# Zylann/godot_atmosphere_shader

Hardware: AMD Instinct MI355X
Metric: Mrays/s, direct32x8 at 1920x1080; 32 view x 8 light steps; % HBM roofline (higher is better)
Workload: dtype f32; 1 GPU; planet_atmosphere_no_clouds, 32 view x 8 light steps (direct light march); 1920x1080; demo scene, pose P_space; width=1920, height=1080, kernel=atmo_render_kernel<4, 8, 1>, gather=none (single GPU)

## Files before the change

### godot_atmosphere_shader_amd/_native.py

```python
from __future__ import annotations

import ctypes as C
import os

from .build import LIB_PATH

ATMO_OK, ATMO_E_NAME, ATMO_E_ARG, ATMO_E_STATE, ATMO_E_HIP, ATMO_E_NO_DEVICE = range(6)
VARIANT_NO_CLOUDS, VARIANT_CLOUDS, VARIANT_CLOUDS_HIGH, VARIANT_CLOUDS_HIGH_RM = range(4)
VARIANT_V1_NO_CLOUDS, VARIANT_V1_CLOUDS, VARIANT_V1_CLOUDS_HIGH = 4, 5, 6
LIGHT_LUT, LIGHT_DIRECT = 0, 1
TEX_2D_R32F, TEX_2D_R8, TEX_3D_R8, TEX_CUBE_R8 = range(4)
MEM_HOST, MEM_DEVICE = 0, 1
ABI_VERSION = 5

CORE_SYMBOLS = (
    "atmo_abi_version", "atmo_device_count", "atmo_create", "atmo_destroy", "atmo_set_param_f32", "atmo_get_param_f32",
    "atmo_set_texture", "atmo_get_texture_size", "atmo_set_sampler_lod", "atmo_bake_optical_depth",
    "atmo_generate_noise_cubemap", "atmo_read_optical_depth", "atmo_render", "atmo_render_composite", "atmo_render_tiles", "atmo_render_tiles_split", "atmo_measure_tile_costs", "atmo_set_precision",
    "atmo_set_host_double_precision", "atmo_set_target_cleared", "atmo_set_tile_feedback", "atmo_last_error_string",
)
DEBUG_SYMBOLS = (
    "atmo_set_lane_split", "atmo_debug_motion_px", "atmo_get_feedback_stats", "atmo_set_timing", "atmo_get_timing", "atmo_host_layout_cubemap", "atmo_host_layout_shape",
    "atmo_host_layout_lut", "atmo_host_cubemap_mip", "atmo_read_texture_layout", "atmo_selftest_exact_math", "atmo_debug_marched_optical_depth", "atmo_debug_log2_cr", "atmo_kernel_name", "atmo_build_id",
    "atmo_get_host_wait_stats", "atmo_get_split_stats", "atmo_debug_create_host_only", "atmo_debug_frame_constants", "atmo_debug_proxy_launch_rect",
    "atmo_debug_store_target", "atmo_debug_views_layout", "atmo_debug_views_proxy_layout", "atmo_debug_tile_order", "atmo_debug_heavy_tile_count", "atmo_debug_feedback_plan",
    "atmo_debug_decode_depth",
)
SCENE_SYMBOLS = ("atmo_render_proxy", "atmo_render_proxy_composite")
TARGET_SYMBOLS = ("atmo_target_pixel_bytes", "atmo_render_target", "atmo_render_proxy_target")
VIEWS_SYMBOLS = ("atmo_render_views",)
MAX_VIEWS = 8
VIEWS_TARGET_SYMBOLS = ("atmo_render_views_target",)
VIEWS_PROXY_SYMBOLS = ("atmo_render_views_proxy", "atmo_render_views_proxy_target")
PLANETS_SYMBOLS = ("atmo_render_planets", "atmo_plan_planets")
MAX_PLANET_DRAWS = 64
DEPTH_SYMBOLS = ("atmo_depth_texel_bytes", "atmo_render_depth_target", "atmo_render_proxy_depth_target", "atmo_render_views_depth_target",
                 "atmo_render_views_proxy_depth_target")
DEPTH_D32_SFLOAT, DEPTH_D16_UNORM, DEPTH_X8_D24_UNORM = range(3)
EXPORTED_SYMBOLS = CORE_SYMBOLS + DEBUG_SYMBOLS + SCENE_SYMBOLS + TARGET_SYMBOLS + VIEWS_SYMBOLS + VIEWS_PROXY_SYMBOLS + VIEWS_TARGET_SYMBOLS
TARGET_RGBA32F, TARGET_RGBA16F, TARGET_RGBA8_UNORM = range(3)
TARGET_RGBA8_SRGB, TARGET_BGRA8_UNORM, TARGET_BGRA8_SRGB, TARGET_A2B10G10R10_UNORM = range(16, 20)


class AtmoFrame(C.Structure):
    _fields_ = [
        ("inv_projection_matrix", C.c_float * 16),
        ("inv_view_matrix", C.c_float * 16),
        ("viewport_w", C.c_int32),
        ("viewport_h", C.c_int32),
        ("planet_center_viewspace", C.c_float * 3),
        ("sun_center_viewspace", C.c_float * 3),
        ("time", C.c_float),
        ("x0", C.c_int32),
        ("y0", C.c_int32),
        ("x1", C.c_int32),
        ("y1", C.c_int32),
    ]


class AtmoTarget(C.Structure):
    _fields_ = [
        ("pixels", C.c_void_p),
        ("format", C.c_int32),
        ("row_pitch_bytes", C.c_int32),
    ]


class AtmoView(C.Structure):
    _fields_ = [
        ("frame", AtmoFrame),
        ("depth_dev", C.c_void_p),
        ("rgba_dev", C.c_void_p),
    ]


class AtmoViewTarget(C.Structure):
    _fields_ = [
        ("frame", AtmoFrame),
        ("depth_dev", C.c_void_p),
        ("target", AtmoTarget),
    ]


class AtmoDepth(C.Structure):
    _fields_ = [
        ("texels", C.c_void_p),
        ("format", C.c_int32),
        ("row_pitch_bytes", C.c_int32),
    ]


class AtmoViewDepthTarget(C.Structure):
    _fields_ = [
        ("frame", AtmoFrame),
        ("depth", AtmoDepth),
        ("target", AtmoTarget),
    ]


class AtmoPlanetDraw(C.Structure):
    _fields_ = [
        ("ctx", C.c_void_p),
        ("frame", AtmoFrame),
        ("model_matrix", C.c_float * 16),
        ("box_size", C.c_float),
        ("depth_dev", C.c_void_p),
        ("target", AtmoTarget),
    ]


class AtmoFeedbackPlanIn(C.Structure):
    _fields_ = [
        ("fb_period", C.c_uint32), ("moving_period", C.c_uint32), ("reach_scale", C.c_float), ("instream", C.c_int32), ("axis_windows", C.c_int32),
        ("cloud_steps", C.c_int32), ("flags", C.c_int32), ("tile_h", C.c_int32), ("batch", C.c_int32), ("n", C.c_uint32), ("last_record", C.c_uint32),
        ("pending", C.c_int32), ("active", C.c_int32), ("order_born", C.c_uint32), ("order_reach_px", C.c_float), ("is_last_n", C.c_uint32),
        ("motion_px", C.c_float), ("sil_px", C.c_float * 2),
    ]


class AtmoFeedbackPlanOut(C.Structure):
    _fields_ = [
# ... 11 lines not shown
_lib = None


def load() -> C.CDLL:
    global _lib
    if _lib is not None:
        return _lib
    if not os.path.exists(LIB_PATH):
        raise RuntimeError(
            f"{LIB_PATH} is missing: the gfx950 HIP extension has not been built "
            "(python -m godot_atmosphere_shader_amd.build). There is no CPU fallback.")
    try:
        import torch
    except ImportError:
        pass
    lib = C.CDLL(LIB_PATH)
    vp, cp, ip, fp = C.c_void_p, C.c_char_p, C.c_int, C.POINTER(C.c_float)
    sig = {
        "atmo_abi_version": (ip, []),
        "atmo_device_count": (ip, []),
        "atmo_create": (ip, [ip, ip, ip, ip, ip, ip, C.POINTER(vp)]),
        "atmo_destroy": (ip, [vp]),
        "atmo_set_param_f32": (ip, [vp, cp, fp, ip]),
        "atmo_get_param_f32": (ip, [vp, cp, fp, ip]),
        "atmo_set_texture": (ip, [vp, cp, ip, ip, ip, ip, ip, vp, ip, vp]),
        "atmo_get_texture_size": (ip, [vp, cp, C.POINTER(ip), C.POINTER(ip), C.POINTER(ip), C.POINTER(ip)]),
        "atmo_set_sampler_lod": (ip, [vp, ip]),
        "atmo_read_texture_layout": (ip, [vp, cp, vp, C.c_size_t, C.POINTER(C.c_size_t), vp]),
        "atmo_host_cubemap_mip": (ip, [vp, ip, vp]),
        "atmo_generate_noise_cubemap": (ip, [vp, ip, C.c_uint32, C.c_float, ip, C.c_float, fp, ip, vp, C.POINTER(C.c_double)]),
        "atmo_bake_optical_depth": (ip, [vp, vp]),
        "atmo_read_optical_depth": (ip, [vp, vp, vp, ip, vp]),
        "atmo_render": (ip, [vp, C.POINTER(AtmoFrame), vp, vp, vp]),
        "atmo_render_composite": (ip, [vp, C.POINTER(AtmoFrame), vp, vp, vp]),
        "atmo_render_tiles": (ip, [vp, C.POINTER(AtmoFrame), vp, vp, vp, ip, vp]),
        "atmo_measure_tile_costs": (ip, [vp, C.POINTER(AtmoFrame), vp, vp, vp, vp, ip, C.POINTER(ip), C.POINTER(ip), C.POINTER(ip), C.POINTER(ip)]),
        "atmo_set_precision": (ip, [vp, ip]),
        "atmo_set_host_double_precision": (ip, [vp, ip]),
        "atmo_set_lane_split": (ip, [vp, ip]),
        "atmo_set_tile_feedback": (ip, [vp, ip]),
        "atmo_set_target_cleared": (ip, [vp, ip]),
        "atmo_debug_motion_px": (C.c_float, [C.POINTER(AtmoFrame), C.POINTER(AtmoFrame), C.c_float, ip]),
        "atmo_get_feedback_stats": (ip, [vp, C.POINTER(ip), C.POINTER(C.c_uint), C.POINTER(C.c_uint), C.POINTER(C.c_uint)]),
        "atmo_set_timing": (ip, [vp, ip]),
        "atmo_get_timing": (ip, [vp, C.POINTER(ip), C.POINTER(C.c_double)]),
        "atmo_selftest_exact_math": (ip, [vp, C.c_uint32, C.c_uint32, C.c_float, C.POINTER(C.c_uint32), C.POINTER(C.c_uint32)]),
        "atmo_debug_marched_optical_depth": (ip, [vp, ip, vp, vp, ip, vp]),
        "atmo_debug_log2_cr": (ip, [vp, ip, vp, vp]),
        "atmo_host_layout_cubemap": (ip, [vp, ip, vp]),
        "atmo_host_layout_shape": (ip, [vp, ip, vp]),
        "atmo_host_layout_lut": (ip, [vp, ip, ip, vp]),
        "atmo_kernel_name": (cp, [vp]),
        "atmo_build_id": (cp, []),
        "atmo_get_host_wait_stats": (ip, [vp, C.POINTER(C.c_uint)]),
        "atmo_get_split_stats": (ip, [vp, C.POINTER(C.c_uint), C.POINTER(C.c_uint)]),
        "atmo_render_tiles_split": (ip, [vp, C.POINTER(AtmoFrame), vp, vp, vp, ip, ip, vp]),
        "atmo_debug_create_host_only": (ip, [ip, ip, ip, ip, ip, C.POINTER(vp)]),
        "atmo_debug_frame_constants": (ip, [vp, C.POINTER(AtmoFrame), ip, C.POINTER(C.c_float), ip, C.POINTER(ip)]),
        "atmo_last_error_string": (cp, [vp]),
        "atmo_debug_proxy_launch_rect": (ip, [vp, C.POINTER(AtmoFrame), fp, C.c_float, C.POINTER(ip), C.POINTER(ip)]),
        "atmo_render_proxy": (ip, [vp, C.POINTER(AtmoFrame), fp, C.c_float, vp, vp, vp]),
        "atmo_render_proxy_composite": (ip, [vp, C.POINTER(AtmoFrame), fp, C.c_float, vp, vp, vp]),
        "atmo_target_pixel_bytes": (ip, [ip]),
        "atmo_render_target": (ip, [vp, C.POINTER(AtmoFrame), vp, C.POINTER(AtmoTarget), ip, vp]),
        "atmo_render_proxy_target": (ip, [vp, C.POINTER(AtmoFrame), fp, C.c_float, vp, C.POINTER(AtmoTarget), ip, vp]),
        "atmo_debug_store_target": (ip, [vp, ip, ip, vp, vp, C.c_size_t, vp]),
        "atmo_render_views": (ip, [vp, C.POINTER(AtmoView), ip, ip, vp]),
        "atmo_debug_views_layout": (ip, [vp, C.POINTER(AtmoView), ip, C.POINTER(ip), C.POINTER(ip)]),
        "atmo_render_views_target": (ip, [vp, C.POINTER(AtmoViewTarget), ip, ip, vp]),
        "atmo_render_views_proxy": (ip, [vp, C.POINTER(AtmoView), ip, fp, C.c_float, ip, vp]),
        "atmo_render_views_proxy_target": (ip, [vp, C.POINTER(AtmoViewTarget), ip, fp, C.c_float, ip, vp]),
        "atmo_debug_views_proxy_layout": (ip, [vp, C.POINTER(AtmoView), ip, fp, C.c_float, C.POINTER(ip), C.POINTER(ip), C.POINTER(ip)]),
        "atmo_render_planets": (ip, [C.POINTER(AtmoPlanetDraw), ip, vp]),
        "atmo_plan_planets": (ip, [C.POINTER(AtmoPlanetDraw), ip, C.POINTER(ip), C.POINTER(ip)]),
        "atmo_depth_texel_bytes": (ip, [ip]),
        "atmo_render_depth_target": (ip, [vp, C.POINTER(AtmoFrame), C.POINTER(AtmoDepth), C.POINTER(AtmoTarget), ip, vp]),
        "atmo_render_proxy_depth_target": (ip, [vp, C.POINTER(AtmoFrame), fp, C.c_float, C.POINTER(AtmoDepth), C.POINTER(AtmoTarget), ip, vp]),
        "atmo_render_views_depth_target": (ip, [vp, C.POINTER(AtmoViewDepthTarget), ip, ip, vp]),
        "atmo_render_views_proxy_depth_target": (ip, [vp, C.POINTER(AtmoViewDepthTarget), ip, fp, C.c_float, ip, vp]),
        "atmo_debug_decode_depth": (ip, [ip, vp, vp, C.c_size_t, vp]),
        "atmo_debug_tile_order": (ip, [vp, vp, ip, ip, ip, ip, vp, vp, vp, vp, C.POINTER(ip)]),
        "atmo_debug_heavy_tile_count": (ip, [vp, ip, ip, C.c_float, C.c_float, ip]),
        "atmo_debug_feedback_plan": (ip, [C.POINTER(AtmoFeedbackPlanIn), C.POINTER(AtmoFeedbackPlanOut)]),
    }
    ab_build = bool(os.environ.get("ATMO_HIP_LIB"))
    for name, (res, args) in sig.items():
        fn = getattr(lib, name, None)
        if fn is None:
            if ab_build:
                continue
            raise RuntimeError(f"libatmo_hip.so does not export {name}; rebuild it")
        fn.restype = res
        fn.argtypes = args
    have = lib.atmo_abi_version()
    if have != ABI_VERSION:
        allowed = {3, 4}
        named = os.environ.get("ATMO_HIP_LIB_ABI", "")
        if not (ab_build and named.isdigit() and int(named) == have and have in allowed):
            raise RuntimeError(f"libatmo_hip.so has ABI version {have}, this binding is written for {ABI_VERSION}; rebuild it"
                               + (f" (an older A/B library needs ATMO_HIP_LIB_ABI={have}; known-compatible: {sorted(allowed)})" if ab_build else ""))
    _lib = lib
    return lib


def check(ctx, code: int) -> None:
    if code != ATMO_OK:
        msg = load().atmo_last_error_string(ctx)
        raise AtmoError(code, msg.decode() if msg else "")
```

### godot_atmosphere_shader_amd/build.py

```python
from __future__ import annotations

import os
import shutil
import subprocess

_HERE = os.path.dirname(os.path.abspath(__file__))
CSRC = os.path.join(_HERE, "csrc")
LIB_PATH = os.environ.get("ATMO_HIP_LIB") or os.path.join(_HERE, "libatmo_hip.so")
SOURCES = ["atmo_api.hip", "atmo_kernels.hip"]
HEADERS = ["atmo_device.h", "atmo_layout.h", "atmo_feedback_plan.h", "atmo_planets_plan.h", "atmo_srgb_tables.h", os.path.join("..", "..", "include", "atmo.h"), os.path.join("..", "..", "include", "atmo_debug.h"),
           os.path.join("..", "..", "include", "atmo_scene.h"), os.path.join("..", "..", "include", "atmo_target.h"),
           os.path.join("..", "..", "include", "atmo_views.h"), os.path.join("..", "..", "include", "atmo_views_target.h"),
           os.path.join("..", "..", "include", "atmo_views_proxy.h"), os.path.join("..", "..", "include", "atmo_planets.h"),
           os.path.join("..", "..", "include", "atmo_depth.h")]

HIPCC_FLAGS = ["--offload-arch=gfx950", "-O3", "-std=c++17", "-ffp-contract=off", "-fno-slp-vectorize", "-fPIC",
               "-shared", "-Wall", "-Wno-unused-function"]


def _hipcc() -> str:
    for cand in (shutil.which("hipcc"), "/opt/rocm/bin/hipcc"):
        if cand and os.path.exists(cand):
            return cand
    raise RuntimeError("hipcc not found: the gfx950 extension cannot be built")


def needs_build() -> bool:
    if not os.path.exists(LIB_PATH):
        return True
    t = os.path.getmtime(LIB_PATH)
    deps = [os.path.join(CSRC, s) for s in SOURCES + HEADERS] + [os.path.abspath(__file__)]
    return any(os.path.getmtime(d) > t for d in deps)


def source_id() -> str:
    import hashlib

    h = hashlib.sha256()
    for name in SOURCES + HEADERS:
        with open(os.path.join(CSRC, name), "rb") as f:
            h.update(name.encode() + b"\0" + f.read())
    h.update(" ".join(HIPCC_FLAGS).encode())
    return h.hexdigest()[:16]


def build_native(force: bool = False, verbose: bool = False) -> str:
    if force or needs_build():
        cmd = [_hipcc()] + HIPCC_FLAGS + [f'-DATMO_BUILD_ID="{source_id()}"', "-o", LIB_PATH] + [os.path.join(CSRC, s) for s in SOURCES]
        if verbose:
            print(" ".join(cmd))
        subprocess.run(cmd, check=True, cwd=CSRC)
    return LIB_PATH


def build_sanitized(verbose: bool = False) -> tuple[str, str]:
    import glob

    lib = os.path.join(_HERE, "libatmo_hip_san.so")
    flags = [f for f in HIPCC_FLAGS if f != "-O3"] + ["-O1", "-g", "-fsanitize=address,undefined", "-fno-sanitize-recover=undefined",
                                                      "-fno-gpu-sanitize", "-shared-libsan"]
    cmd = [_hipcc()] + flags + ["-o", lib] + [os.path.join(CSRC, s) for s in SOURCES]
    if verbose:
        print(" ".join(cmd))
    subprocess.run(cmd, check=True, cwd=CSRC)
    rt = sorted(glob.glob("/opt/rocm/lib/llvm/lib/clang/*/lib/linux/libclang_rt.asan-x86_64.so"))
    if not rt:
        raise RuntimeError("the ASan runtime of ROCm's clang was not found")
    return lib, rt[-1]


if __name__ == "__main__":
    import sys

    if "--sanitize" in sys.argv:
        print(*build_sanitized(verbose=True))
    else:
        print(build_native(force=True, verbose=True))
```

### godot_atmosphere_shader_amd/csrc/atmo_api.hip

```cpp
#include "../../include/atmo.h"
#include "../../include/atmo_debug.h"
#include "../../include/atmo_scene.h"
#include "../../include/atmo_target.h"
#include "../../include/atmo_views.h"
#include "../../include/atmo_views_target.h"
#include "../../include/atmo_views_proxy.h"
#include "../../include/atmo_planets.h"
#include "../../include/atmo_depth.h"
#include "atmo_device.h"
#include "atmo_layout.h"
#include "atmo_feedback_plan.h"
#include "atmo_planets_plan.h"
#include "atmo_srgb_tables.h"

#include <array>
#include <cmath>
#include <cstdio>
#include <cstdlib>
#include <cstring>
#include <limits>
#include <new>
#include <string>
#include <vector>

namespace {

struct ParamDesc {
    const char *name;
    int count;
    size_t offset;
};

struct Params {
    float u_planet_radius = 1.0f;
    float u_atmosphere_height = 0.1f;
    float u_sun_position[3] = {0, 0, 0};
    float u_density = 0.2f;
    float u_scattering_strength = 20.0f;
    float u_scattering_wavelengths[3] = {700, 530, 440};
    float u_atmosphere_modulate[3] = {1, 1, 1};
    float u_atmosphere_ambient_color[3] = {0, 0, 0.002f / 12.92f};
    float u_clip_mode = 0.0f;
    float u_sphere_depth_factor = 0.0f;
    float u_cloud_density_scale = 50.0f;
    float u_cloud_bottom = 0.2f;
    float u_cloud_top = 0.5f;
    float u_cloud_blend = 0.5f;
    float u_world_to_model_matrix[16] = {1, 0, 0, 0, 0, 1, 0, 0, 0, 0, 1, 0, 0, 0, 0, 1};
    float u_cloud_shape_invert = 0.0f;
    float u_cloud_coverage_bias = 0.0f;
    float u_cloud_shape_factor = 0.8f;
    float u_cloud_shape_scale = 1.0f;
    float u_cloud_coverage_rotation[4] = {1, 0, 0, 1};
    float u_day_color0[4] = {0.21404114f, 0.60382734f, 1.0f, 1.0f};
    float u_day_color1[4] = {0.21404114f, 0.60382734f, 1.0f, 1.0f};
    float u_night_color0[4] = {0.03310477f, 0.13286832f, 0.60382734f, 1.0f};
    float u_night_color1[4] = {0.03310477f, 0.13286832f, 0.60382734f, 1.0f};
    float u_day_night_transition_scale = 2.0f;
};

#define PD(field, n) {#field, n, offsetof(Params, field)}
const ParamDesc kParams[] = {
    PD(u_planet_radius, 1), PD(u_atmosphere_height, 1), PD(u_sun_position, 3), PD(u_density, 1),
    PD(u_scattering_strength, 1), PD(u_scattering_wavelengths, 3), PD(u_atmosphere_modulate, 3),
    PD(u_atmosphere_ambient_color, 3), PD(u_clip_mode, 1), PD(u_sphere_depth_factor, 1),
    PD(u_cloud_density_scale, 1), PD(u_cloud_bottom, 1), PD(u_cloud_top, 1), PD(u_cloud_blend, 1),
    PD(u_world_to_model_matrix, 16), PD(u_cloud_shape_invert, 1), PD(u_cloud_coverage_bias, 1),
    PD(u_cloud_shape_factor, 1), PD(u_cloud_shape_scale, 1), PD(u_cloud_coverage_rotation, 4),
    PD(u_day_color0, 4), PD(u_day_color1, 4), PD(u_night_color0, 4), PD(u_night_color1, 4),
    PD(u_day_night_transition_scale, 1),
};
#undef PD

const ParamDesc *find_param(const char *name) {
    if (!name) return nullptr;
    for (const ParamDesc &d : kParams)
        if (std::strcmp(d.name, name) == 0) return &d;
    return nullptr;
}

struct DeviceBuffer {
    void *ptr = nullptr;
    size_t bytes = 0;
};

constexpr int F4_MAX_CUBE_N = 1024, F4_MAX_SHAPE_N = 64;

thread_local std::string g_create_error = "";

}

// ... 1 lines not shown
    int device = 0;
    int variant = 0;
    int flags = 0;
    int view_steps = 8, cloud_steps = 0, light_steps = 0;
    Params p;
    DeviceBuffer lut, blue, shape, cube;
    DeviceBuffer cube_f4, shape_f4;
    int f4_max_shape_n = F4_MAX_SHAPE_N;
    DeviceBuffer lut4;
    int lut_w = 0, lut_h = 0, shape_n = 0, cube_n = 0;
    int cube_levels = 0;
    DeviceBuffer cube_level_off;
    uint32_t cube_level_off_host[16] = {0};
    int sampler_lod = -1;
    DeviceBuffer staging;
    hipStream_t staging_stream = nullptr;
    bool staging_used = false;
    hipEvent_t tex_event = nullptr;
    hipStream_t tex_stream = nullptr;
    bool tex_pending = false;
    unsigned tex_version = 0;
    hipStream_t tex_waited_stream = nullptr;
    unsigned tex_waited_version = 0;
    int host_double_precision = 0;
    int target_cleared = 0;
    int lane_split = 0;
    int last_split = 1;
    int last_flags = -1;
    int tile_feedback = -1;
    struct FeedbackState {
        bool used = false;
        int tiles_x = 0, tiles_y = 0, split = 0;
        hipStream_t draw_stream = nullptr;
        DeviceBuffer cost, order[2];
        DeviceBuffer dil[2];
        AtmoFrame prev_frame;
        bool have_prev = false;
        float motion_px = 0.0f;
        float sil_px[2] = {0.0f, 0.0f};
        float order_reach_px[2] = {0.0f, 0.0f};
        unsigned order_born[2] = {0, 0};
        DeviceBuffer is_order, is_scratch;
        unsigned is_last_n = ~0u;
        DeviceBuffer order2[2], is_order2;
        uint32_t *class_totals = nullptr;
        unsigned n = 0;
        unsigned last_record = 0;
        int active = -1;
        int write = 0;
        bool pending = false;
        bool drop_pending = false;
        hipEvent_t ev_draw = nullptr, ev_order[2] = {nullptr, nullptr};
        unsigned long long last_use = 0;
        bool dirty = false;
    };
    struct GeoCache {
        float key[26] = {0};
        int rows = -1;
        uint16_t prefix[atmo::GEO_MAX_ROWS + 1];
        uint8_t first[atmo::GEO_MAX_ROWS];
        uint16_t hint[2][atmo::GEO_MAX_HINTS + 2];
    } geo;
    int geo_order = 1;
    unsigned geo_draws = 0;
    static constexpr int FB_SLOTS = 4;
    FeedbackState fb[FB_SLOTS];
    unsigned long long fb_clock = 0;
    int fb_budget = 8;
    unsigned fb_ordered_draws = 0, fb_recycled = 0, fb_sorts = 0;
    hipStream_t fb_stream = nullptr;
    hipStream_t split_stream = nullptr;
    int heavy_split = 1;
    float heavy_split_trigger = 2.0f;
    float heavy_split_trigger_moving = 2.0f;
    float heavy_split_ratio = 0.3f;
    unsigned split_draws = 0, split_tiles_last = 0;
    DeviceBuffer fb_scratch;
    unsigned fb_period = 8;
    int env_feedback = -1, env_split = 0;
    float env_reach_scale = 1.0f;
    unsigned moving_period = 2;
    int f4_footprints = 3;
    int env_lod0_cert = 1;
    int instream = 1;
    int fb_axis_windows = 1;
    uint32_t *measure_cost = nullptr;
    struct DrawStream { hipStream_t stream = nullptr; hipEvent_t last_draw = nullptr; bool recorded = false; unsigned long long last_use = 0; };
    unsigned long long draw_stream_clock = 0;
    std::vector<DrawStream> draw_streams;
    bool draw_streams_many = false;
    int draw_events = 1;
    hipEvent_t xs_event[8] = {nullptr};
    unsigned xs_next = 0;
    unsigned device_syncs = 0;
    DeviceBuffer measure_buf;
    struct TileListBuf { hipStream_t stream = nullptr; DeviceBuffer buf; bool used = false; unsigned long long last_use = 0; } tile_lists[4];
    unsigned long long tile_list_clock = 0;
#ifdef ATMO_WAVE_TRACE
    DeviceBuffer wave_trace;
    size_t wave_trace_waves = 0;
#endif
    static constexpr int VIEWS_RING = 16;
    struct ViewsSlot {
        atmo::RenderConsts *host = nullptr;
        atmo::RenderConsts *dev = nullptr;
        hipEvent_t done = nullptr;
        bool in_flight = false;
    } views_ring[VIEWS_RING];
    atmo::RenderConsts *views_host = nullptr;
    DeviceBuffer views_dev;
    unsigned views_next = 0;
    unsigned views_ring_waits = 0;
    FeedbackState views_fb;
    struct ViewsFeedbackKey {
        int flags = -1, n = 0, grid[8][2] = {{0}};
        AtmoFrame prev[8];
        float motion_px[8] = {0};
    } views_key;
    int timing = 0;
    int launch_counter = 0;
    int timed_launches = 0;
    double timed_ms = 0.0;
    std::vector<std::pair<hipEvent_t, hipEvent_t>> pending;
    std::string err;
};

namespace {

int fail(AtmoContext *ctx, int code, const std::string &msg) {
    if (ctx) ctx->err = msg; else g_create_error = msg;
    return code;
}

int hip_fail(AtmoContext *ctx, hipError_t e, const char *what) {
    return fail(ctx, ATMO_E_HIP, std::string(what) + ": " + hipGetErrorString(e));
}

#define HIP_TRY(ctx, call)                                   \
    do {                                                     \
        hipError_t e_ = (call);                              \
        if (e_ != hipSuccess) return hip_fail(ctx, e_, #call); \
    } while (0)

#define ATMO_TRY(call) do { const int rc_ = (call); if (rc_ != ATMO_OK) return rc_; } while (0)

int dev_alloc(AtmoContext *ctx, DeviceBuffer &b, size_t bytes) {
    if (b.ptr && b.bytes == bytes) return ATMO_OK;
    if (b.ptr) { (void)hipFree(b.ptr); b.ptr = nullptr; b.bytes = 0; }
    if (bytes == 0) return ATMO_OK;
    HIP_TRY(ctx, hipMalloc(&b.ptr, bytes));
    b.bytes = bytes;
    return ATMO_OK;
}

void dev_free(DeviceBuffer &b) {
    if (b.ptr) (void)hipFree(b.ptr);
    b.ptr = nullptr;
    b.bytes = 0;
}

void build_cube_footprints(const uint8_t *faces, int n, std::vector<uint32_t> &out) {
    const int fs = n + 1;
    out.assign((size_t)6 * fs * fs, 0u);
    for (int f = 0; f < 6; ++f)
        for (int j = 0; j < fs; ++j)
            for (int i = 0; i < fs; ++i) out[((size_t)f * fs + j) * fs + i] = atmo::cube_footprint_word(faces, n, f, i, j);
}

void build_shape_footprints(const uint8_t *t, int n, std::vector<uint32_t> &out) {
    out.assign((size_t)n * n * n, 0u);
    for (int k = 0; k < n; ++k)
        for (int j = 0; j < n; ++j)
            for (int i = 0; i < n; ++i) out[((size_t)k * n + j) * n + i] = atmo::shape_footprint_word(t, n, i, j, k);
}

void build_lut_apron(const float *lut, int w, int h, std::vector<float> &out) {
    const int st = w + 2;
    out.assign((size_t)st * (h + 2), 0.0f);
    for (int j = 0; j < h + 2; ++j)
        for (int i = 0; i < st; ++i) out[(size_t)j * st + i] = atmo::lut_apron_value(lut, w, h, i, j);
}

inline float pow2f(float x) { return x * x; }
inline float pow4f(float x) { return x * x * x * x; }
inline float mixf(float a, float b, float t) { return a * (1.0f - t) + b * t; }
inline float clampf(float x, float lo, float hi) { return std::fmin(std::fmax(x, lo), hi); }
inline float smoothstepf(float e0, float e1, float x) {
    float t = clampf((x - e0) / (e1 - e0), 0.0f, 1.0f);
    return t * t * (3.0f - 2.0f * t);
}

void fill_consts(const AtmoContext *ctx, const AtmoFrame *f, const float *depth, float *rgba, atmo::RenderConsts &rc) {
    const Params &p = ctx->p;
    std::memset(&rc, 0, sizeof(rc));
    std::memcpy(rc.inv_p, f->inv_projection_matrix, sizeof(rc.inv_p));
    std::memcpy(rc.inv_v, f->inv_view_matrix, sizeof(rc.inv_v));
    const float *V = f->inv_view_matrix;
    for (int r = 0; r < 3; ++r) rc.cam_pos_world[r] = V[0 + r] * 0.0f + V[4 + r] * 0.0f + V[8 + r] * 0.0f + V[12 + r] * 1.0f;
    rc.vw = (float)f->viewport_w;
    rc.vh = (float)f->viewport_h;
    rc.rcp_vw = 1.0f / rc.vw;
    rc.rcp_vh = 1.0f / rc.vh;
    rc.w = f->viewport_w; rc.h = f->viewport_h;
    rc.x0 = f->x0; rc.y0 = f->y0; rc.x1 = f->x1; rc.y1 = f->y1;
    for (int i = 0; i < 3; ++i) rc.center[i] = f->planet_center_viewspace[i];
    {
        float d[3];
        for (int i = 0; i < 3; ++i) d[i] = f->sun_center_viewspace[i] - f->planet_center_viewspace[i];
        float inv = 1.0f / std::sqrt(d[0] * d[0] + d[1] * d[1] + d[2] * d[2]);
        for (int i = 0; i < 3; ++i) rc.sun_dir[i] = d[i] * inv;
    }
    rc.planet_radius = p.u_planet_radius;
    rc.atmosphere_height = p.u_atmosphere_height;
    rc.atmosphere_radius = p.u_planet_radius + p.u_atmosphere_height;
    rc.density = p.u_density;
    rc.sphere_depth_factor = p.u_sphere_depth_factor;
    for (int i = 0; i < 3; ++i) {
        rc.coeff[i] = pow4f(400.0f / p.u_scattering_wavelengths[i]) * p.u_scattering_strength;
        rc.ambient[i] = p.u_atmosphere_ambient_color[i];
        rc.modulate[i] = p.u_atmosphere_modulate[i];
    }
    rc.view_steps = ctx->view_steps;
    rc.light_steps = ctx->light_steps;
    for (int i = 0; i < 3; ++i) {
        rc.day0[i] = p.u_day_color0[i]; rc.day1[i] = p.u_day_color1[i];
        rc.night0[i] = p.u_night_color0[i]; rc.night1[i] = p.u_night_color1[i];
    }
    rc.day_night_transition_scale = p.u_day_night_transition_scale;

    rc.clouds_bottom = p.u_planet_radius + p.u_cloud_bottom * p.u_atmosphere_height;
    rc.clouds_top = p.u_planet_radius + p.u_cloud_top * p.u_atmosphere_height;
    rc.cloud_thickness = rc.clouds_top - rc.clouds_bottom;
    rc.inv_cloud_thickness = 1.0f / rc.cloud_thickness;
    {
        const double lo = (double)rc.clouds_bottom * (double)rc.clouds_bottom * (1.0 - 2e-6);
        const double hi = (double)rc.clouds_top * (double)rc.clouds_top * (1.0 + 2e-6);
        rc.layer_r2_lo = (float)lo;
        rc.layer_r2_hi = (float)hi;
        if (!(rc.clouds_bottom > 0.0f)) rc.layer_r2_lo = 0.0f;
        if (!(rc.cloud_thickness > 0.0f) || !(rc.clouds_top > 0.0f) || !std::isfinite(rc.layer_r2_hi)) { rc.layer_r2_lo = 0.0f; rc.layer_r2_hi = INFINITY; }
    }
    rc.cloud_density_scale = p.u_cloud_density_scale;
    rc.cloud_blend = p.u_cloud_blend;
    rc.coverage_bias = p.u_cloud_coverage_bias;
    rc.shape_factor = p.u_cloud_shape_factor;
    rc.shape_scale = p.u_cloud_shape_scale;
    rc.shape_invert = (p.u_cloud_shape_invert == 1.0f) ? 1 : 0;
    {
        const float f = p.u_cloud_shape_factor;
        const float t_hi = 1.0f + 9.5367431640625e-07f;
        float a = 0.5f * (1.0f - f) + 0.0f * f, b = 0.5f * (1.0f - f) + t_hi * f;
        if (rc.shape_invert) { a = 1.0f - a; b = 1.0f - b; }
        rc.shape_lo01 = std::fmin(a, b) - 0.1f;
        rc.shape_hi01 = std::fmax(a, b) - 0.1f;
    }
    std::memcpy(rc.cov_rot, p.u_cloud_coverage_rotation, sizeof(rc.cov_rot));
    const float *A = p.u_world_to_model_matrix;
    for (int col = 0; col < 4; ++col)
        for (int row = 0; row < 4; ++row)
            rc.view_to_model[col * 4 + row] = A[0 * 4 + row] * V[col * 4 + 0] + A[1 * 4 + row] * V[col * 4 + 1] +
                                              A[2 * 4 + row] * V[col * 4 + 2] + A[3 * 4 + row] * V[col * 4 + 3];
    const float *M = rc.view_to_model;
    for (int r = 0; r < 3; ++r) {
        rc.origin_model[r] = M[0 + r] * 0.0f + M[4 + r] * 0.0f + M[8 + r] * 0.0f + M[12 + r] * 1.0f;
        rc.sun_dir_model[r] = M[0 + r] * rc.sun_dir[0] + M[4 + r] * rc.sun_dir[1] + M[8 + r] * rc.sun_dir[2] + M[12 + r] * 0.0f;
    }
    {
        const float ground = p.u_planet_radius, top = rc.clouds_top, bottom = rc.clouds_bottom;
        const float space = 0.5f * std::sqrt(1.0f - pow2f(ground / top)) * bottom;
        const float groundd = 3.0f * space;
        const float len = std::sqrt(rc.origin_model[0] * rc.origin_model[0] + rc.origin_model[1] * rc.origin_model[1] +
                                    rc.origin_model[2] * rc.origin_model[2]);
        rc.max_d = mixf(groundd, space, smoothstepf(bottom, top * 1.05f, len));
    }
    rc.cloud_steps = ctx->cloud_steps;
    rc.inv_cloud_steps = ctx->cloud_steps > 0 ? 1.0f / (float)ctx->cloud_steps : 0.0f;
    {
        const float reach = (rc.clouds_top - rc.clouds_bottom) * 0.15f;
        const float inv_steps = 1.0f / 6.0f;
        float step_len = reach * inv_steps;
        for (int i = 0; i < 6; ++i) {
            rc.rm_offset[i] = (float)i * step_len;
            rc.rm_weight[i] = step_len * p.u_cloud_density_scale;
            for (int c = 0; c < 3; ++c) rc.rm_tap[i][c] = rc.rm_offset[i] * rc.sun_dir_model[c];
            step_len *= 1.2f;
        }
    }
    rc.lut = (const float *)ctx->lut.ptr; rc.lut_w = ctx->lut_w; rc.lut_h = ctx->lut_h;
    rc.lut4 = (const float *)ctx->lut4.ptr;
    rc.blue = (const uint8_t *)ctx->blue.ptr;
    rc.shape = (const uint32_t *)ctx->shape.ptr; rc.shape_n = ctx->shape_n;
    rc.shape_log2n = -1;
    for (int b = 0; b < 10; ++b) if (ctx->shape_n == (1 << b)) rc.shape_log2n = b;
    rc.cube = (const uint32_t *)ctx->cube.ptr; rc.cube_n = ctx->cube_n;
    rc.cube_levels = ctx->cube_levels;
    rc.cube_level_off = (const uint32_t *)ctx->cube_level_off.ptr;
    rc.cube_bytes = (uint32_t)ctx->cube.bytes;
    rc.cube_f4 = (ctx->f4_footprints & 1) ? (const float *)ctx->cube_f4.ptr : nullptr;
    rc.shape_f4 = (ctx->f4_footprints & 2) ? (const float *)ctx->shape_f4.ptr : nullptr;
    rc.cube_lod_fast = (ctx->cube_n >= 1 && ctx->cube_n <= 1024 && (ctx->cube_n & (ctx->cube_n - 1)) == 0) ? 1 : 0;
    {
        rc.lod0_inv_c = std::numeric_limits<float>::infinity();
        rc.lod0_last = (float)(rc.cloud_steps - 1);
        rc.lod0_drift = (float)((rc.cloud_steps + 1) * 2.07e-7);
        const double n = (double)ctx->cube_n;
        const double a = rc.cov_rot[0], b = rc.cov_rot[2], c = rc.cov_rot[1], d = rc.cov_rot[3];
        const double fro = a * a + b * b + c * c + d * d, det = a * d - b * c;
        const double disc = fro * fro - 4.0 * det * det;
        const double sigma = std::sqrt(0.5 * (fro + std::sqrt(disc > 0.0 ? disc : 0.0))) * (1.0 + 1e-6);
        const double sigma_min = sigma > 0.0 ? std::fabs(det) / sigma : 0.0;
        const double sigma_eff = sigma > 1.0 ? sigma : 1.0;
        if (rc.cube_lod_fast && ctx->cube_n >= 4 && sigma <= 2.0 && sigma_min >= 0.5) {
            rc.lod0_inv_c = (float)(1.0 / (0.97 * 4.0 * (1.0 - 2.0 / n) * (1.0 - 2.0 / n) / (n * n * sigma_eff * sigma_eff)));
        }
        if (ctx->env_lod0_cert == 0) rc.lod0_inv_c = std::numeric_limits<float>::infinity();
    }
    {
        const float *Pm = f->inv_projection_matrix;
        const double cc = (double)rc.center[0] * rc.center[0] + (double)rc.center[1] * rc.center[1] + (double)rc.center[2] * rc.center[2];
        const double k = cc - (double)rc.atmosphere_radius * rc.atmosphere_radius;
        const bool depth_free = Pm[8] == 0.0f && Pm[9] == 0.0f && Pm[10] == 0.0f;
        rc.miss_k = (depth_free && k > 0.01 * cc && std::isfinite(k)) ? (float)(k * (1.0 - 1e-3) * (1.0 - 1e-3)) : 0.0f;
    }
    rc.depth = depth;
    rc.out = (float4 *)rgba;
    rc.out_pitch = f->x1 - f->x0;
    rc.out_x0 = f->x0;
    rc.out_y0 = f->y0;
    rc.composite = 0;
    rc.store_discards = ctx->target_cleared ? 0 : 1;
    rc.gx0 = f->x0;
    rc.gy0 = f->y0;
}

int resolve_sampler_lod(const AtmoContext *ctx, const char **why_not) {
    if (why_not) *why_not = nullptr;
    if (ctx->sampler_lod == 0 || !(ctx->flags & atmo::KF_CLOUDS) || !ctx->cube.ptr || ctx->cube_levels <= 1) return 0;
    if (!(ctx->flags & atmo::KF_PRECISE)) {
        if (why_not) *why_not = "atmo_render: the implicit cubemap LOD (atmo_set_sampler_lod 1) needs the precise cloud mode (atmo_set_precision 1)";
        return 0;
    }
    return 1;
}

int heavy_tile_count(const uint32_t *totals, int n_tiles, float ratio, float trigger, int resident_waves) {
    double life[atmo::TILE_ORDER_CLASSES], sum = 0.0;
    long long counted = 0;
    for (int k = 0; k < atmo::TILE_ORDER_CLASSES; ++k) {
        constexpr int P = atmo::TILE_ORDER_PER_OCTAVE;
        const int q = atmo::TILE_ORDER_CLASSES - 1 - k + 8 * P;
        life[k] = P == 2 ? std::ldexp(1.0, q >> 1) * ((q & 1) ? 1.5 : 1.0) * 1.2
                         : std::ldexp(1.0, q / P) * (1.0 + ((q % P) + 0.5) / P);
        if (k == atmo::TILE_ORDER_CLASSES - 1) life[k] = 0.0;
        sum += life[k] * (double)totals[k];
        counted += totals[k];
    }
    if (counted != n_tiles || sum <= 0.0) return 0;
    const double draw = sum * 2.0 / (double)resident_waves;
    int first = 0;
    while (first < atmo::TILE_ORDER_CLASSES - 1 && totals[first] == 0) ++first;
    if (!(life[first] > trigger * draw)) return 0;
    int heavy = 0;
    for (int k = 0; k < atmo::TILE_ORDER_CLASSES && life[k] > ratio * draw; ++k) heavy += (int)totals[k];
    return heavy > n_tiles / 3 ? n_tiles / 3 : heavy;
}

int choose_split(const AtmoContext *ctx, const AtmoFrame *f) {
    (void)f;
    if (ctx->flags & atmo::KF_ATMO_REF) return 1;
    if (ctx->env_split) return ctx->env_split;
    return ctx->lane_split == 2 ? 2 : 1;
}

void launch_shape(const AtmoContext *ctx, const AtmoFrame *frame, int *flags_out, int *split_out, bool *lod_out) {
    int flags = ctx->flags, split = choose_split(ctx, frame);
    if (ctx->view_steps > 32 && !(flags & (atmo::KF_LITE | atmo::KF_ATMO_REF))) {
        flags |= atmo::KF_VIEW_POS;
        split = 1;
    }
    const bool lod = resolve_sampler_lod(ctx, nullptr) != 0;
    if (lod) {
        flags |= atmo::KF_CUBE_LOD;
        if ((flags & ~atmo::KF_CLOUD_LIGHT_RM) != (atmo::KF_CUBE_LOD | atmo::KF_PRECISE | atmo::KF_CLOUDS)) split = 1;
    }
    *flags_out = flags;
    *split_out = split;
    if (lod_out) *lod_out = lod;
}

int check_frame(AtmoContext *ctx, const std::string &who, const AtmoFrame *frame, bool *empty) {
    if (!frame) return fail(ctx, ATMO_E_ARG, who + ": null frame");
    if (frame->viewport_w < 1 || frame->viewport_h < 1 || frame->viewport_w > 65536 || frame->viewport_h > 65536)
        return fail(ctx, ATMO_E_ARG, who + ": bad viewport size");
    if (frame->x0 < 0 || frame->y0 < 0 || frame->x1 > frame->viewport_w || frame->y1 > frame->viewport_h ||
        frame->x0 > frame->x1 || frame->y0 > frame->y1)
        return fail(ctx, ATMO_E_ARG, who + ": rect outside the viewport");
    *empty = frame->x0 == frame->x1 || frame->y0 == frame->y1;
    return ATMO_OK;
}
int check_draw_pointers(AtmoContext *ctx, const std::string &who, const float *depth_dev, const float *rgba_dev, bool float4_target) {
    if (!depth_dev || !rgba_dev) return fail(ctx, ATMO_E_ARG, who + ": null device pointer");
    if (float4_target && (reinterpret_cast<uintptr_t>(rgba_dev) & 15u) != 0) return fail(ctx, ATMO_E_ARG, who + ": rgba_dev must be 16-byte aligned");
    return ATMO_OK;
}
static_assert((int)ATMO_DEPTH_D32_SFLOAT == (int)atmo::DF_D32_SFLOAT && (int)ATMO_DEPTH_D16_UNORM == (int)atmo::DF_D16_UNORM &&
                  (int)ATMO_DEPTH_X8_D24_UNORM == (int)atmo::DF_X8_D24_UNORM,
              "DepthFormat == AtmoDepthFormat");
int depth_check(AtmoContext *ctx, const std::string &who, const AtmoDepth *depth, int w, int h, atmo::DepthConsts *out) {
    (void)h;
    if (!depth) return fail(ctx, ATMO_E_ARG, who + ": null depth");
    const int tb = atmo::depth_texel_bytes(depth->format);
    if (tb == 0) return fail(ctx, ATMO_E_ARG, who + ": unknown depth format " + std::to_string(depth->format));
    if (!depth->texels) return fail(ctx, ATMO_E_ARG, who + ": null depth texels");
    if ((reinterpret_cast<uintptr_t>(depth->texels) & (uintptr_t)(tb - 1)) != 0)
        return fail(ctx, ATMO_E_ARG, who + ": depth texels must be aligned to the texel size (" + std::to_string(tb) + " bytes)");
// ... 352 lines not shown
bool two_lane_form(const AtmoContext *ctx, int flags) {
    const int lod_cloud = atmo::KF_CUBE_LOD | atmo::KF_PRECISE | atmo::KF_CLOUDS;
    return ctx->heavy_split == 2 ? (flags & ~atmo::KF_CLOUD_LIGHT_RM) == lod_cloud : flags == (lod_cloud | atmo::KF_CLOUD_LIGHT_RM);
}

}

extern "C" {

int atmo_abi_version(void) { return ATMO_ABI_VERSION; }
#ifndef ATMO_BUILD_ID
#define ATMO_BUILD_ID "unstamped"
#endif
const char *atmo_build_id(void) { return ATMO_BUILD_ID; }

int atmo_device_count(void) {
    int n = 0;
    hipError_t e = hipGetDeviceCount(&n);
    if (e != hipSuccess) return -ATMO_E_NO_DEVICE;
    return n;
}

static int check_create_args(int variant, int view_steps, int cloud_steps, int light_mode, int light_steps, AtmoContext **out) {
    if (!out) return fail(nullptr, ATMO_E_ARG, "atmo_create: out is null");
    *out = nullptr;
    if (variant < ATMO_VARIANT_NO_CLOUDS || variant > ATMO_VARIANT_V1_CLOUDS_HIGH)
        return fail(nullptr, ATMO_E_ARG, "atmo_create: unknown variant");
    if (light_mode != ATMO_LIGHT_LUT && light_mode != ATMO_LIGHT_DIRECT)
        return fail(nullptr, ATMO_E_ARG, "atmo_create: unknown light mode");
    if (view_steps < 0 || view_steps > 4096 || cloud_steps < 0 || cloud_steps > 4096 || light_steps < 0 || light_steps > 4096)
        return fail(nullptr, ATMO_E_ARG, "atmo_create: step count out of range");
    if (light_mode == ATMO_LIGHT_DIRECT && light_steps < 1)
        return fail(nullptr, ATMO_E_ARG, "atmo_create: direct light mode needs light_steps >= 1");
    return ATMO_OK;
}
static void init_variant(AtmoContext *ctx, int device, int variant, int view_steps, int cloud_steps, int light_mode, int light_steps) {
    ctx->device = device;
    ctx->variant = variant;
    const bool lite = variant >= ATMO_VARIANT_V1_NO_CLOUDS;
    static const int shipped_cloud_steps[7] = {0, 32, 64, 64, 0, 32, 64};
    ctx->view_steps = view_steps > 0 ? view_steps : (lite ? 16 : 8);
    ctx->cloud_steps = shipped_cloud_steps[variant] == 0 ? 0 : (cloud_steps > 0 ? cloud_steps : shipped_cloud_steps[variant]);
    ctx->light_steps = (light_mode == ATMO_LIGHT_DIRECT && !lite) ? light_steps : 0;
    ctx->flags = 0;
    if (ctx->cloud_steps > 0) ctx->flags |= atmo::KF_CLOUDS | atmo::KF_PRECISE;
    if (lite) ctx->flags |= atmo::KF_PRECISE;
    if (variant == ATMO_VARIANT_CLOUDS_HIGH_RM) ctx->flags |= atmo::KF_CLOUD_LIGHT_RM;
    if (light_mode == ATMO_LIGHT_DIRECT && !lite) ctx->flags |= atmo::KF_LIGHT_DIRECT;
    if (lite) ctx->flags |= atmo::KF_LITE;
}

int atmo_create(int device, int variant, int view_steps, int cloud_steps, int light_mode, int light_steps,
                AtmoContext **out) {
    ATMO_TRY(check_create_args(variant, view_steps, cloud_steps, light_mode, light_steps, out));
    int n = 0;
    hipError_t e = hipGetDeviceCount(&n);
    if (e != hipSuccess || n <= 0)
        return fail(nullptr, ATMO_E_NO_DEVICE, std::string("atmo_create: no HIP device (") + hipGetErrorString(e) + ")");
    if (device < 0 || device >= n) return fail(nullptr, ATMO_E_NO_DEVICE, "atmo_create: device index out of range");
    hipDeviceProp_t prop;
    e = hipGetDeviceProperties(&prop, device);
    if (e != hipSuccess) return hip_fail(nullptr, e, "hipGetDeviceProperties");
    if (std::strncmp(prop.gcnArchName, "gfx950", 6) != 0)
        return fail(nullptr, ATMO_E_NO_DEVICE, std::string("atmo_create: device is ") + prop.gcnArchName + ", this library is built for gfx950 only");
    e = hipSetDevice(device);
    if (e != hipSuccess) return hip_fail(nullptr, e, "hipSetDevice");

    AtmoContext *ctx = new (std::nothrow) AtmoContext();
    if (!ctx) return fail(nullptr, ATMO_E_ARG, "atmo_create: out of host memory");
    init_variant(ctx, device, variant, view_steps, cloud_steps, light_mode, light_steps);

    if (const char *ev = std::getenv("ATMO_LANE_SPLIT")) ctx->env_split = ev[0] == '1' ? 1 : (ev[0] == '2' ? 2 : 0);
    if (const char *ev = std::getenv("ATMO_TILE_FEEDBACK")) ctx->env_feedback = ev[0] == '1' ? 1 : 0;
    if (const char *ev = std::getenv("ATMO_F4")) ctx->f4_footprints = std::atoi(ev) & 3;
    if (const char *ev = std::getenv("ATMO_F4_SHAPE_MAX")) ctx->f4_max_shape_n = std::atoi(ev);
    if (const char *ev = std::getenv("ATMO_LOD0_CERT")) ctx->env_lod0_cert = ev[0] == '0' ? 0 : 1;
    if (const char *ev = std::getenv("ATMO_HEAVY_SPLIT")) ctx->heavy_split = ev[0] == '0' ? 0 : (ev[0] == '2' ? 2 : 1);
    if (const char *ev = std::getenv("ATMO_HEAVY_SPLIT_RATIO")) ctx->heavy_split_ratio = (float)std::atof(ev);
    if (const char *ev = std::getenv("ATMO_HEAVY_SPLIT_TRIGGER")) ctx->heavy_split_trigger = (float)std::atof(ev);
    if (const char *ev = std::getenv("ATMO_HEAVY_SPLIT_TRIGGER_MOVING")) ctx->heavy_split_trigger_moving = (float)std::atof(ev);
    if (const char *ev = std::getenv("ATMO_DRAW_EVENTS")) ctx->draw_events = ev[0] == '0' ? 0 : (ev[0] == '2' ? 2 : 1);
    if (const char *ev = std::getenv("ATMO_TARGET_CLEARED")) ctx->target_cleared = ev[0] == '1' ? 1 : 0;
    if (const char *ev = std::getenv("ATMO_GEO_ORDER")) ctx->geo_order = ev[0] == '0' ? 0 : 1;
    if (const char *ev = std::getenv("ATMO_FB_INSTREAM")) ctx->instream = ev[0] >= '1' && ev[0] <= '2' ? ev[0] - '0' : 0;
    if (const char *ev = std::getenv("ATMO_FB_AXIS_WINDOWS")) ctx->fb_axis_windows = ev[0] == '1' ? 1 : 0;
    if (const char *ev = std::getenv("ATMO_FB_REACH_SCALE")) ctx->env_reach_scale = (float)std::atof(ev);
    if (const char *ev = std::getenv("ATMO_FB_MOVING_PERIOD")) { const int v = std::atoi(ev); ctx->moving_period = (unsigned)(v < 1 ? 1 : v); }
    if (const char *ev = std::getenv("ATMO_TILE_FEEDBACK_PERIOD")) { const int v = std::atoi(ev); ctx->fb_period = (unsigned)(v < 1 ? 1 : v); }

    int rc = dev_alloc(ctx, ctx->blue, 256 * 256);
    if (rc == ATMO_OK) {
        e = hipMemset(ctx->blue.ptr, 0, 256 * 256);
        if (e != hipSuccess) rc = hip_fail(ctx, e, "hipMemset");
    }
    if (rc != ATMO_OK) {
        g_create_error = ctx->err;
        dev_free(ctx->blue);
        delete ctx;
        return rc;
    }
    *out = ctx;
    return ATMO_OK;
}

int atmo_destroy(AtmoContext *ctx) {
    if (!ctx) return ATMO_OK;
    if (ctx->device < 0) { delete ctx; return ATMO_OK; }
    (void)hipSetDevice(ctx->device);
    drain_timing(ctx);
    dev_free(ctx->lut);
    dev_free(ctx->lut4);
    dev_free(ctx->blue);
    dev_free(ctx->shape);
    dev_free(ctx->cube);
    dev_free(ctx->cube_level_off);
    dev_free(ctx->cube_f4);
    dev_free(ctx->shape_f4);
    dev_free(ctx->staging);
    dev_free(ctx->measure_buf);
    for (AtmoContext::TileListBuf &t : ctx->tile_lists) dev_free(t.buf);
    if (ctx->tex_event) (void)hipEventDestroy(ctx->tex_event);
    for (hipEvent_t &ev : ctx->xs_event) if (ev) (void)hipEventDestroy(ev);
    for (AtmoContext::DrawStream &d : ctx->draw_streams) if (d.last_draw) (void)hipEventDestroy(d.last_draw);

    if (ctx->fb_stream) {
        (void)hipStreamSynchronize(ctx->fb_stream);
        (void)hipStreamDestroy(ctx->fb_stream);
    }
    if (ctx->split_stream) {
        (void)hipStreamSynchronize(ctx->split_stream);
        (void)hipStreamDestroy(ctx->split_stream);
    }
    for (int i = 0; i <= AtmoContext::FB_SLOTS; ++i) {
        AtmoContext::FeedbackState &f = i < AtmoContext::FB_SLOTS ? ctx->fb[i] : ctx->views_fb;
        if (f.ev_draw) (void)hipEventDestroy(f.ev_draw);
        for (int k = 0; k < 2; ++k) {
            if (f.ev_order[k]) (void)hipEventDestroy(f.ev_order[k]);
            dev_free(f.order[k]);
            dev_free(f.dil[k]);
        }
        dev_free(f.is_order);
        dev_free(f.is_scratch);
        dev_free(f.is_order2);
        for (int k = 0; k < 2; ++k) dev_free(f.order2[k]);
        if (f.class_totals) (void)hipHostFree(f.class_totals);
        dev_free(f.cost);
    }
    for (AtmoContext::ViewsSlot &v : ctx->views_ring) {
        if (v.done) { (void)hipEventSynchronize(v.done); (void)hipEventDestroy(v.done); }
    }
    if (ctx->views_host) (void)hipHostFree(ctx->views_host);
    dev_free(ctx->views_dev);
    dev_free(ctx->fb_scratch);
    delete ctx;
    return ATMO_OK;
}

int atmo_set_param_f32(AtmoContext *ctx, const char *name, const float *v, int n) {
    if (!ctx) return ATMO_E_ARG;
    if (!v) return fail(ctx, ATMO_E_ARG, "atmo_set_param_f32: value is null");
    const ParamDesc *d = find_param(name);
    if (!d) return fail(ctx, ATMO_E_NAME, std::string("atmo_set_param_f32: unknown uniform '") + (name ? name : "(null)") + "'");
    if (n != d->count)
        return fail(ctx, ATMO_E_ARG, std::string("atmo_set_param_f32: '") + name + "' takes " + std::to_string(d->count) + " floats");
    std::memcpy(reinterpret_cast<char *>(&ctx->p) + d->offset, v, sizeof(float) * n);
    return ATMO_OK;
// ... 824 lines not shown
    if (e != hipSuccess) return hip_fail(ctx, e, "atmo_debug_marched_optical_depth");
    return ATMO_OK;
}

int atmo_debug_log2_cr(AtmoContext *ctx, int n, const float *x, float *out) {
    if (!ctx) return ATMO_E_ARG;
    if (n < 1 || !x || !out) return fail(ctx, ATMO_E_ARG, "atmo_debug_log2_cr: bad argument");
    HIP_TRY(ctx, hipSetDevice(ctx->device));
    float *d = nullptr;
    HIP_TRY(ctx, hipMalloc(&d, 2 * (size_t)n * sizeof(float)));
    hipError_t e = hipMemcpy(d, x, (size_t)n * sizeof(float), hipMemcpyHostToDevice);
    if (e == hipSuccess) e = atmo::launch_log2_cr(d, d + n, n, nullptr);
    if (e == hipSuccess) e = hipMemcpy(out, d + n, (size_t)n * sizeof(float), hipMemcpyDeviceToHost);
    (void)hipFree(d);
    if (e != hipSuccess) return hip_fail(ctx, e, "atmo_debug_log2_cr");
    return ATMO_OK;
}

int atmo_debug_tile_order(AtmoContext *ctx, const uint32_t *cost, int tiles_x, int tiles_y, int rx, int ry, uint32_t *order_out, uint32_t *order2_out,
                          uint32_t *class_totals_out, uint32_t *cost_after_out, int *n_classes_out) {
    if (!ctx) return ATMO_E_ARG;
    if (!cost || !order_out) return fail(ctx, ATMO_E_ARG, "atmo_debug_tile_order: cost and order_out must not be NULL");
    if (tiles_x < 1 || tiles_y < 1 || (long long)tiles_x * tiles_y > (1ll << 22))
        return fail(ctx, ATMO_E_ARG, "atmo_debug_tile_order: the grid must be at least 1 x 1 and hold at most 2^22 tiles");
    if (rx < 0 || ry < 0 || rx > 64 || ry > 64) return fail(ctx, ATMO_E_ARG, "atmo_debug_tile_order: dilation radii are 0 .. 64 tiles");
    HIP_TRY(ctx, hipSetDevice(ctx->device));
    constexpr size_t NC = atmo::TILE_ORDER_CLASSES;
    const size_t n = (size_t)tiles_x * (size_t)tiles_y, scratch_words = atmo::tile_order_scratch_bytes() / sizeof(uint32_t);
    const size_t words = 6 * n + NC + scratch_words;
    uint32_t *d = nullptr;
    HIP_TRY(ctx, hipMalloc(&d, words * sizeof(uint32_t)));
    uint32_t *d_cost = d, *d_order = d + n, *d_order2 = d + 2 * n, *d_tmp1 = d + 4 * n, *d_tmp2 = d + 5 * n, *d_totals = d + 6 * n, *d_scratch = d_totals + NC;
    hipError_t e = hipMemset(d, 0xFF, words * sizeof(uint32_t));
    if (e == hipSuccess) e = hipMemcpy(d_cost, cost, n * sizeof(uint32_t), hipMemcpyHostToDevice);
    if (e == hipSuccess) e = atmo::launch_tile_order(d_cost, d_order, tiles_x, tiles_y, rx, ry, d_tmp1, d_tmp2, d_scratch, nullptr,
                                                     order2_out ? d_order2 : nullptr, class_totals_out ? d_totals : nullptr);
    if (e == hipSuccess) e = hipMemcpy(order_out, d_order, n * sizeof(uint32_t), hipMemcpyDeviceToHost);
    if (e == hipSuccess && order2_out) e = hipMemcpy(order2_out, d_order2, 2 * n * sizeof(uint32_t), hipMemcpyDeviceToHost);
    if (e == hipSuccess && class_totals_out) e = hipMemcpy(class_totals_out, d_totals, NC * sizeof(uint32_t), hipMemcpyDeviceToHost);
    if (e == hipSuccess && cost_after_out) e = hipMemcpy(cost_after_out, d_cost, n * sizeof(uint32_t), hipMemcpyDeviceToHost);
    (void)hipFree(d);
    if (e != hipSuccess) return hip_fail(ctx, e, "atmo_debug_tile_order");
    if (n_classes_out) *n_classes_out = (int)NC;
    return ATMO_OK;
}

int atmo_debug_heavy_tile_count(const uint32_t *class_totals, int n_classes, int n_tiles, float ratio, float trigger, int resident_waves) {
    if (!class_totals || n_classes != atmo::TILE_ORDER_CLASSES || n_tiles < 0 || resident_waves < 1)
        return -fail(nullptr, ATMO_E_ARG, "atmo_debug_heavy_tile_count: bad argument (NULL totals, a class count other than the build's, n_tiles < 0 or resident_waves < 1)");
    return heavy_tile_count(class_totals, n_tiles, ratio, trigger, resident_waves);
}

const char *atmo_kernel_name(AtmoContext *ctx) {
    if (!ctx) return "";
    if (ctx->last_flags >= 0) return atmo::render_kernel_name(ctx->last_flags, ctx->light_steps, ctx->last_split);
    int flags = 0, split = 1;
    launch_shape(ctx, nullptr, &flags, &split, nullptr);
    return atmo::render_kernel_name(flags, ctx->light_steps, split);
}

const char *atmo_last_error_string(AtmoContext *ctx) {
    if (!ctx) return g_create_error.c_str();
    return ctx->err.c_str();
}

int atmo_get_split_stats(AtmoContext *ctx, unsigned *split_draws, unsigned *heavy_tiles_last) {
    if (!ctx) return ATMO_E_ARG;
    if (split_draws) *split_draws = ctx->split_draws;
    if (heavy_tiles_last) *heavy_tiles_last = ctx->split_tiles_last;
    return ATMO_OK;
}

int atmo_get_host_wait_stats(AtmoContext *ctx, unsigned *device_syncs) {
    if (!ctx) return ATMO_E_ARG;
    if (device_syncs) *device_syncs = ctx->device_syncs;
    return ATMO_OK;
}

int atmo_debug_create_host_only(int variant, int view_steps, int cloud_steps, int light_mode, int light_steps, AtmoContext **out) {
    ATMO_TRY(check_create_args(variant, view_steps, cloud_steps, light_mode, light_steps, out));
    AtmoContext *ctx = new (std::nothrow) AtmoContext();
    if (!ctx) return fail(nullptr, ATMO_E_ARG, "atmo_debug_create_host_only: out of host memory");
    init_variant(ctx,  -1, variant, view_steps, cloud_steps, light_mode, light_steps);
    *out = ctx;
    return ATMO_OK;
}

int atmo_debug_frame_constants(AtmoContext *ctx, const AtmoFrame *frame, int cube_n, float *out, int capacity, int *count) {
    if (!ctx) return ATMO_E_ARG;
    if (!frame) return fail(ctx, ATMO_E_ARG, "atmo_debug_frame_constants: null frame");
    if (cube_n < 0 || cube_n > 4096) return fail(ctx, ATMO_E_ARG, "atmo_debug_frame_constants: bad cubemap size");
    const int saved_n = ctx->cube_n;
    ctx->cube_n = cube_n;
    AtmoFrame fixed;
    atmo::RenderConsts rc;
    fill_consts(ctx, draw_frame(ctx, frame, fixed), nullptr, nullptr, rc);
    ctx->cube_n = saved_n;
    std::vector<float> v;
    auto put = [&](const float *p, int n) { v.insert(v.end(), p, p + n); };
    auto put1 = [&](float x) { v.push_back(x); };
    put(rc.cam_pos_world, 3); put(rc.sun_dir, 3); put1(rc.atmosphere_radius); put(rc.coeff, 3);
    put1(rc.clouds_bottom); put1(rc.clouds_top); put1(rc.cloud_thickness); put1(rc.inv_cloud_thickness);
    put1(rc.layer_r2_lo); put1(rc.layer_r2_hi); put1(rc.shape_lo01); put1(rc.shape_hi01);
    put(rc.view_to_model, 16); put(rc.origin_model, 3); put(rc.sun_dir_model, 3);
    put1(rc.max_d); put1(rc.inv_cloud_steps); put(rc.rm_offset, 6); put(rc.rm_weight, 6); put(&rc.rm_tap[0][0], 18);
    put1(rc.lod0_inv_c); put1(rc.lod0_last); put1(rc.lod0_drift); put1(rc.miss_k); put1(rc.rcp_vw); put1(rc.rcp_vh);
    put1((float)rc.shape_invert); put1((float)rc.cube_lod_fast); put1((float)rc.store_discards);
    if (count) *count = (int)v.size();
    if (!out) return ATMO_OK;
    if (capacity < (int)v.size()) return fail(ctx, ATMO_E_ARG, "atmo_debug_frame_constants: buffer too small");
    std::memcpy(out, v.data(), v.size() * sizeof(float));
    return ATMO_OK;
}


static void mat4_mul_d(const double *a, const double *b, double *c) {
    for (int col = 0; col < 4; ++col)
        for (int row = 0; row < 4; ++row) {
            double acc = 0.0;
            for (int k = 0; k < 4; ++k) acc += a[k * 4 + row] * b[col * 4 + k];
            c[col * 4 + row] = acc;
        }
}
static bool mat4_inverse_d(const double *m, double *inv) {
    double a[4][8];
    for (int r = 0; r < 4; ++r)
        for (int c = 0; c < 4; ++c) { a[r][c] = m[c * 4 + r]; a[r][c + 4] = r == c ? 1.0 : 0.0; }
    for (int c = 0; c < 4; ++c) {
        int piv = c;
        for (int r = c + 1; r < 4; ++r) if (std::fabs(a[r][c]) > std::fabs(a[piv][c])) piv = r;
        if (!(std::fabs(a[piv][c]) > 0.0) || !std::isfinite(a[piv][c])) return false;
        for (int k = 0; k < 8; ++k) std::swap(a[c][k], a[piv][k]);
        const double d = a[c][c];
        for (int k = 0; k < 8; ++k) a[c][k] /= d;
        for (int r = 0; r < 4; ++r)
            if (r != c && a[r][c] != 0.0) {
                const double f = a[r][c];
                for (int k = 0; k < 8; ++k) a[r][k] -= f * a[c][k];
            }
    }
    for (int r = 0; r < 4; ++r)
        for (int c = 0; c < 4; ++c) inv[c * 4 + r] = a[r][c + 4];
    return true;
}

static int proxy_setup(AtmoContext *ctx, const char *who, const AtmoFrame *f, const float *model_matrix, float box_size, bool lod,
                       atmo::ProxyConsts &pc, int rect[4], int *tiles_x, int *tiles_y) {
    double ip[16], iv[16], m[16], mi[16], v[16], p[16], t[16], k[16], pv[16];
    for (int i = 0; i < 16; ++i) { ip[i] = f->inv_projection_matrix[i]; iv[i] = f->inv_view_matrix[i]; m[i] = model_matrix[i]; }
    if (!mat4_inverse_d(m, mi)) return fail(ctx, ATMO_E_ARG, std::string(who) + ": model_matrix is singular");
    if (!mat4_inverse_d(iv, v)) return fail(ctx, ATMO_E_ARG, std::string(who) + ": inv_view_matrix is singular");
    if (!mat4_inverse_d(ip, p)) return fail(ctx, ATMO_E_ARG, std::string(who) + ": inv_projection_matrix is singular");
    mat4_mul_d(mi, iv, t);
    mat4_mul_d(t, ip, k);
    for (int r = 0; r < 4; ++r)
        for (int c = 0; c < 4; ++c) pc.k[r][c] = (float)k[c * 4 + r];
    const double h = 0.5 * (double)box_size;
    pc.half = (float)h;
    mat4_mul_d(v, m, t);
    mat4_mul_d(p, t, pv);
    double eye[4] = {k[8], k[9], k[10], k[11]};
    bool eye_point = std::fabs(eye[3]) > 1e-12 * (std::fabs(eye[0]) + std::fabs(eye[1]) + std::fabs(eye[2]));
    if (eye_point) {
        for (int r = 0; r < 3; ++r) eye[r] /= eye[3];
    } else {
        double dn[3], df[3];
        for (int r = 0; r < 3; ++r) { dn[r] = (k[8 + r] + k[12 + r]) / (k[11] + k[15]); df[r] = k[12 + r] / k[15]; }
        if (eye[0] * (df[0] - dn[0]) + eye[1] * (df[1] - dn[1]) + eye[2] * (df[2] - dn[2]) > 0.0)
            for (int r = 0; r < 3; ++r) eye[r] = -eye[r];
    }
    const double W = f->viewport_w, H = f->viewport_h;
    double xmin = INFINITY, xmax = -INFINITY, ymin = INFINITY, ymax = -INFINITY;
    bool unbounded = false;
    for (int face = 0; face < 6; ++face) {
        const int ax = face >> 1;
        const double sg = (face & 1) ? -1.0 : 1.0;
        if (!(sg * eye[ax] > (eye_point ? h : 0.0))) continue;
        const int u = (ax + 1) % 3, w3 = (ax + 2) % 3;
        std::vector<std::array<double, 4>> poly, next;
        for (int c = 0; c < 4; ++c) {
            double mp[3];
            mp[ax] = sg * h;
            mp[u] = (c == 1 || c == 2) ? h : -h;
            mp[w3] = (c >= 2) ? h : -h;
            std::array<double, 4> q;
            for (int r = 0; r < 4; ++r) q[r] = pv[0 * 4 + r] * mp[0] + pv[1 * 4 + r] * mp[1] + pv[2 * 4 + r] * mp[2] + pv[3 * 4 + r];
            poly.push_back(q);
        }
        const double side[4] = {2.0 * ((double)f->x0 + 0.49) / W - 1.0, 2.0 * ((double)f->x1 - 0.49) / W - 1.0,
                                2.0 * ((double)f->y0 + 0.49) / H - 1.0, 2.0 * ((double)f->y1 - 0.49) / H - 1.0};
        for (int pl = 0; pl < 6 && !poly.empty(); ++pl) {
            auto g = [pl, &side](const std::array<double, 4> &q) {
                switch (pl) {
                case 0: return q[2];
                case 1: return q[3] - q[2];
                case 2: return q[0] - side[0] * q[3];
                case 3: return side[1] * q[3] - q[0];
// ... 785 lines not shown
```

### godot_atmosphere_shader_amd/csrc/atmo_device.h

```cpp
#pragma once

#include <hip/hip_runtime.h>
#include <stdint.h>

namespace atmo {

constexpr int GEO_MAX_ROWS = 272;
constexpr int GEO_MAX_HINTS = 256;
struct RenderConsts {
    float inv_p[16];
    float inv_v[16];
    float cam_pos_world[3];
    float vw, vh;
    int32_t w, h;
    int32_t x0, y0, x1, y1;
    float center[3];
    float sun_dir[3];
    float planet_radius, atmosphere_height;
    float atmosphere_radius;
    float density;
    float sphere_depth_factor;
    float coeff[3];
    float ambient[3], modulate[3];
    int32_t view_steps;
    int32_t light_steps;
    float day0[3], day1[3], night0[3], night1[3];
    float day_night_transition_scale;
    float clouds_bottom, clouds_top;
    float cloud_thickness;
    float inv_cloud_thickness;
    float layer_r2_lo, layer_r2_hi;
    float cloud_density_scale, cloud_blend, coverage_bias, shape_factor, shape_scale;
    int32_t shape_invert;
    float shape_lo01, shape_hi01;
    float cov_rot[4];
    float view_to_model[16];
    float origin_model[3];
    float sun_dir_model[3];
    float max_d;
    float inv_cloud_steps;
    int32_t cloud_steps;
    float rm_offset[6];
    float rm_weight[6];
    float rm_tap[6][3];
    const float *lut;
    int32_t lut_w, lut_h;
    const float *lut4;
    const uint8_t *blue;
    const uint32_t *shape;
    int32_t shape_n;
    int32_t shape_log2n;
    const uint32_t *cube;
    int32_t cube_n;
    int32_t cube_levels;
    const uint32_t *cube_level_off;
    uint32_t cube_bytes;
    int32_t cube_lod_fast;
    float lod0_inv_c;
    float lod0_last, lod0_drift;
    const float *depth;
    float4 *out;
    int32_t out_pitch;
    int32_t out_x0, out_y0;
    int32_t composite;
    int32_t tiles_x;
    const uint32_t *tile_order;
    uint32_t *tile_cost;
#ifdef ATMO_WAVE_TRACE
    unsigned long long *wave_trace;
#endif
    float rcp_vw, rcp_vh;
    const float *cube_f4;
    const float *shape_f4;
    float miss_k;
    int32_t gx0, gy0;
    int32_t store_discards;
    int32_t cost_rows_halved;
    int32_t geo_rows;
    uint16_t geo_prefix[GEO_MAX_ROWS + 1];
    uint8_t geo_first[GEO_MAX_ROWS];
    uint16_t geo_hint[2][GEO_MAX_HINTS + 2];
};

struct BakeConsts {
    float planet_radius, atmosphere_height, density;
    int32_t w, h, steps;
    float *out;
};

struct NoiseCubemapConsts {
    int32_t resolution;
    uint32_t seed;
    float frequency, gain;
    int32_t octaves;
    float scale[3];
    uint8_t *out;
};

enum KernelFlags : int { KF_CLOUDS = 1, KF_CLOUD_LIGHT_RM = 2, KF_LIGHT_DIRECT = 4, KF_LITE = 8, KF_PRECISE = 16, KF_CUBE_LOD = 32,
                          KF_ATMO_REF = 64 ,
                          KF_VIEW_POS = 128 ,
                          KF_GEO = 256 ,
                          KF_PROXY = 512 ,
                          KF_TARGET = 1024 ,
                          KF_VIEWS = 2048 ,
                          KF_DEPTH = 4096  };

struct ProxyConsts {
    float k[4][4];
    float half;
};

enum TargetFormat : int { TF_RGBA32F = 0, TF_RGBA16F = 1, TF_RGBA8_UNORM = 2,
                          TF_RGBA8_SRGB = 16, TF_BGRA8_UNORM = 17, TF_BGRA8_SRGB = 18, TF_A2B10G10R10_UNORM = 19 };
inline bool target_format_packed(int format) { return format == TF_RGBA16F || format == TF_RGBA8_UNORM || (format >= TF_RGBA8_SRGB && format <= TF_A2B10G10R10_UNORM); }
struct TargetConsts {
    void *pixels;
    int32_t pitch_bytes;
    int32_t format;
};

enum DepthFormat : int { DF_D32_SFLOAT = 0, DF_D16_UNORM = 1, DF_X8_D24_UNORM = 2 };
inline int depth_texel_bytes(int format) { return format == DF_D16_UNORM ? 2 : (format == DF_D32_SFLOAT || format == DF_X8_D24_UNORM) ? 4 : 0; }
struct DepthConsts {
    const void *texels;
    int32_t pitch_bytes;
    int32_t format;
};

constexpr int MAX_VIEWS = 8;
struct ViewsConsts {
    uint32_t first_block[MAX_VIEWS + 1];
    const uint32_t *order;
    uint32_t *cost;
};
struct ViewsTargetConsts {
    ViewsConsts v;
    TargetConsts target[MAX_VIEWS];
};
struct ViewsProxyConsts {
    uint32_t first_block[MAX_VIEWS + 1];
    ProxyConsts proxy[MAX_VIEWS];
};
struct ViewsProxyTargetConsts {
    ViewsProxyConsts p;
    TargetConsts target[MAX_VIEWS];
};

struct ViewsDepthConsts {
    DepthConsts depth[MAX_VIEWS];
};

hipError_t launch_render(int flags, int split, const RenderConsts &rc, hipStream_t stream, int tile_list_blocks = 0);
bool default_family_supported(int flags);
hipError_t launch_render_proxy(int flags, const RenderConsts &rc, const ProxyConsts &pc, hipStream_t stream);
hipError_t launch_render_views(int flags, int light_steps, const RenderConsts *table_dev, const ViewsConsts &vc, hipStream_t stream);
hipError_t launch_render_views_target(int flags, int light_steps, const RenderConsts *table_dev, const ViewsTargetConsts &vtc, hipStream_t stream);
hipError_t launch_render_views_proxy(int flags, int light_steps, const RenderConsts *table_dev, const ViewsProxyConsts &vpc, hipStream_t stream);
hipError_t launch_render_views_proxy_target(int flags, int light_steps, const RenderConsts *table_dev, const ViewsProxyTargetConsts &vptc, hipStream_t stream);
bool target_family_supported(int flags, int split);
hipError_t launch_render_target(int flags, int split, const RenderConsts &rc, const TargetConsts &tc, hipStream_t stream, int tile_list_blocks = 0);
hipError_t launch_render_proxy_target(int flags, const RenderConsts &rc, const ProxyConsts &pc, const TargetConsts &tc, hipStream_t stream);
hipError_t launch_render_depth_target(int flags, int split, const RenderConsts &rc, const TargetConsts &tc, const DepthConsts &dc, hipStream_t stream,
                                      int tile_list_blocks = 0);
// ... 37 lines not shown
```

### godot_atmosphere_shader_amd/csrc/atmo_kernels.hip

```cpp
#include "atmo_device.h"
#include "atmo_layout.h"
#include "atmo_srgb_tables.h"

#include <cstdio>
#include <type_traits>

namespace atmo {

#ifndef ATMO_TILE_H
#define ATMO_TILE_H 8
#endif
constexpr int TILE_W = 16;
constexpr int TILE_H = ATMO_TILE_H;
#ifndef ATMO_WAVE_W
#define ATMO_WAVE_W 16
#endif
constexpr int WAVE_W = ATMO_WAVE_W;
constexpr int WAVE_H = 64 / WAVE_W;
static_assert(WAVE_W == 16 || WAVE_W == 8 || WAVE_W == 32, "wave tile");
constexpr float LOG2E = 1.44269504088896340736f;

__device__ __forceinline__ float hw_exp2(float x) { return __builtin_amdgcn_exp2f(x); }
__device__ __forceinline__ float hw_rsq(float x) { return __builtin_amdgcn_rsqf(x); }
#ifndef ATMO_LOD_LAMBDA_EXACT
#define ATMO_LOD_LAMBDA_EXACT 1
#endif
#ifndef ATMO_RCP_NR
#define ATMO_RCP_NR 1
#endif
#ifndef ATMO_LOD_LOG2_CR
#define ATMO_LOD_LOG2_CR 1
#endif
__device__ __forceinline__ float hw_rcp(float x) { return __builtin_amdgcn_rcpf(x); }
__device__ __forceinline__ float hw_sqrt(float x) { return __builtin_amdgcn_sqrtf(x); }
__device__ __forceinline__ float sat(float x) { return __builtin_amdgcn_fmed3f(x, 0.0f, 1.0f); }
__device__ __forceinline__ float clampf(float x, float lo, float hi) { return fminf(fmaxf(x, lo), hi); }
__device__ __forceinline__ float mixf(float a, float b, float t) { return a * (1.0f - t) + b * t; }
__device__ __forceinline__ float ieee_sqrt(float x) { return __builtin_sqrtf(x); }
__device__ __forceinline__ float ieee_div(float a, float b) { return a / b; }
__device__ __forceinline__ float exact_rcp(float d) {
    float r = hw_rcp(d);
#pragma unroll
    for (int k = 0; k < ATMO_RCP_NR; ++k) r = __builtin_fmaf(__builtin_fmaf(-d, r, 1.0f), r, r);
    return r;
}

__device__ __forceinline__ float exact_sqrt(float x) {
    const float s = hw_sqrt(x);
    const float s_dn = __int_as_float(__float_as_int(s) - 1);
    const float s_up = __int_as_float(__float_as_int(s) + 1);
    const float r_dn = __builtin_fmaf(-s_dn, s, x);
    const float r_up = __builtin_fmaf(-s_up, s, x);
    float o = (r_dn <= 0.0f) ? s_dn : s;
    o = (r_up > 0.0f) ? s_up : o;
    return o;
}
__device__ __forceinline__ float exact_sqrt_pos(float x) {
    const float y = hw_rsq(x);
    float g = x * y, h = 0.5f * y;
    const float e = __builtin_fmaf(-h, g, 0.5f);
    h = __builtin_fmaf(h, e, h);
    g = __builtin_fmaf(g, e, g);
    const float d = __builtin_fmaf(-g, g, x);
    return __builtin_fmaf(d, h, g);
}
__device__ __forceinline__ float exact_div_uniform(float a, float c, float rc) {
    const float q0 = a * rc;
    const float q1 = __builtin_fmaf(__builtin_fmaf(-q0, c, a), rc, q0);
    return __builtin_fmaf(__builtin_fmaf(-q1, c, a), rc, q1);
}

#ifndef ATMO_FAST_MISS_MASK
#define ATMO_FAST_MISS_MASK 0x05
#endif
#ifndef ATMO_DIRECT_PROLOGUE_DIET
#define ATMO_DIRECT_PROLOGUE_DIET 1
#endif
template <bool DIET = true>
__device__ __forceinline__ float prologue_sqrt(float x) { return DIET ? exact_sqrt(x) : ieee_sqrt(x); }
template <bool DIET = true>
__device__ __forceinline__ float pixel_coord(float a, float n, float rcp_n) {
    if (!DIET) return ieee_div(a, n);
    const float q0 = a * rcp_n;
    return __builtin_fmaf(__builtin_fmaf(-q0, n, a), rcp_n, q0);
}
template <bool DIET = true>
__device__ __forceinline__ void world_div3(float wx, float wy, float wz, float ww, float &x, float &y, float &z) {
    const float aw = fabsf(ww);
    if (DIET && aw >= 7.8886090522101181e-31f && aw <= 1.2676506002282294e30f) {
        const float rw = ieee_div(1.0f, ww);
        x = exact_div_uniform(wx, ww, rw);
        y = exact_div_uniform(wy, ww, rw);
        z = exact_div_uniform(wz, ww, rw);
    } else {
        x = ieee_div(wx, ww); y = ieee_div(wy, ww); z = ieee_div(wz, ww);
    }
}
template <bool DIET = true>
__device__ __forceinline__ float blue_noise_value(uint8_t b);

__device__ __forceinline__ float swap_adjacent(float x) {
    return __int_as_float(__builtin_amdgcn_update_dpp(0, __float_as_int(x), 0xB1, 0xF, 0xF, true));
}

__device__ __forceinline__ float swap_across_quads(float x) {
    const int v = __float_as_int(x);
    int t = __builtin_amdgcn_update_dpp(v, v, 0x104, 0xF, 0x5, false);
    t = __builtin_amdgcn_update_dpp(t, v, 0x114, 0xF, 0xA, false);
    return __int_as_float(t);
}
template <bool ACROSS_QUADS>
__device__ __forceinline__ float swap_ray_lanes(float x) { return ACROSS_QUADS ? swap_across_quads(x) : swap_adjacent(x); }
__device__ __forceinline__ float mul_unfused(float a, float b) { return a * b; }
__device__ __forceinline__ float add_unfused(float a, float b) { return a + b; }
__device__ __forceinline__ float sub_unfused(float a, float b) { return a - b; }

struct V3 {
    float x, y, z;
};
__device__ __forceinline__ float dot_lr(V3 a, V3 b) { return a.x * b.x + a.y * b.y + a.z * b.z; }

struct SphereHit {
    float b;
    float qc2;
};
__device__ __forceinline__ SphereHit sphere_setup(V3 center, V3 dir) {
    V3 oc = {0.0f - center.x, 0.0f - center.y, 0.0f - center.z};
    float b = dot_lr(oc, dir);
    V3 qc = {oc.x - b * dir.x, oc.y - b * dir.y, oc.z - b * dir.z};
    SphereHit s;
    s.b = b;
    s.qc2 = dot_lr(qc, qc);
    return s;
}
template <bool DIET = true>
__device__ __forceinline__ float2 hit_radius(SphereHit s, float radius) {
    float h = radius * radius - s.qc2;
    if (h < 0.0f) return make_float2(1000000.0f, 1000000.0f);
    h = prologue_sqrt<DIET>(h);
    return make_float2(-s.b - h, -s.b + h);
}


typedef float f32x2 __attribute__((ext_vector_type(2)));
__device__ __forceinline__ __amdgpu_buffer_rsrc_t make_rsrc(const void *base, uint32_t bytes) {
    return __builtin_amdgcn_make_buffer_rsrc(const_cast<void *>(base), 0, (int)bytes, 0x00020000);
}
#ifndef ATMO_ABLATE_FETCH
#define ATMO_ABLATE_FETCH 0
#endif
#if ATMO_ABLATE_FETCH
#define ATMO_ABLATED_F32 0.50196081399917603f
__device__ __forceinline__ uint32_t buf_u32(__amdgpu_buffer_rsrc_t, uint32_t byte_off) {
    asm volatile("" : "+v"(byte_off));
    return 0x80808080u;
}
__device__ __forceinline__ f32x2 buf_f32x2(__amdgpu_buffer_rsrc_t, uint32_t byte_off) {
    asm volatile("" : "+v"(byte_off));
    return f32x2{ATMO_ABLATED_F32, ATMO_ABLATED_F32};
}
#else
__device__ __forceinline__ uint32_t buf_u32(__amdgpu_buffer_rsrc_t r, uint32_t byte_off) {
    return (uint32_t)__builtin_amdgcn_raw_buffer_load_b32(r, (int)byte_off, 0, 0);
}
__device__ __forceinline__ f32x2 buf_f32x2(__amdgpu_buffer_rsrc_t r, uint32_t byte_off) {
    return __builtin_bit_cast(f32x2, __builtin_amdgcn_raw_buffer_load_b64(r, (int)byte_off, 0, 0));
}
#endif

__device__ __forceinline__ float ub0(uint32_t w) { return (float)(w & 0xffu); }
__device__ __forceinline__ float ub1(uint32_t w) { return (float)((w >> 8) & 0xffu); }
__device__ __forceinline__ float ub2(uint32_t w) { return (float)((w >> 16) & 0xffu); }
__device__ __forceinline__ float ub3(uint32_t w) { return (float)(w >> 24); }

typedef float f32x4 __attribute__((ext_vector_type(4)));
#if ATMO_ABLATE_FETCH
__device__ __forceinline__ f32x4 buf_f32x4(__amdgpu_buffer_rsrc_t, uint32_t byte_off) {
    asm volatile("" : "+v"(byte_off));
    return f32x4{ATMO_ABLATED_F32, ATMO_ABLATED_F32, ATMO_ABLATED_F32, ATMO_ABLATED_F32};
}
#else
__device__ __forceinline__ f32x4 buf_f32x4(__amdgpu_buffer_rsrc_t r, uint32_t byte_off) {
    return __builtin_bit_cast(f32x4, __builtin_amdgcn_raw_buffer_load_b128(r, (int)byte_off, 0, 0));
}
#endif
__device__ __forceinline__ float lut_sample_fp(const float *__restrict__ lut4, int w1, int h1, float x, float y) {
#pragma clang fp contract(fast)
    const float xf = floorf(x), yf = floorf(y);
    const float fx = x - xf, fy = y - yf;
    const __amdgpu_buffer_rsrc_t rs = make_rsrc(lut4, (uint32_t)(w1 * h1) * 16u);
    const float s16 = (float)(w1 * 16);
    const uint32_t off = (uint32_t)fmaf(yf, s16, fmaf(xf, 16.0f, s16 + 16.0f));
    const f32x4 t = buf_f32x4(rs, off);
    const float a = t.x + (t.y - t.x) * fx;
    const float b = t.z + (t.w - t.z) * fx;
    return a + (b - a) * fy;
}

__device__ __forceinline__ float trilinear_exact8(f32x4 a, f32x4 b, float fx, float fy, float fz) {
    const float gx = 1.0f - fx, gy = 1.0f - fy, gz = 1.0f - fz;
    const float c00 = a.x * gx + a.y * fx;
    const float c10 = a.z * gx + a.w * fx;
    const float c01 = b.x * gx + b.y * fx;
    const float c11 = b.z * gx + b.w * fx;
    const float c0 = c00 * gy + c10 * fy;
    const float c1 = c01 * gy + c11 * fy;
    return c0 * gz + c1 * fz;
}
__device__ __forceinline__ float unorm8_exact(float b);

struct ShapeAddr {
    uint32_t e0, e1;
};
__device__ __forceinline__ int wrap_general(int i, int n, float nf, float inv_nf) {
    const int q = (int)floorf((float)i * inv_nf);
    int r = i - q * n;
    r = r < 0 ? r + n : r;
    return r >= n ? r - n : r;
}
__device__ __forceinline__ ShapeAddr shape_addr(int n, int log2n, int i, int j, int k) {
// ... 544 lines not shown
        lod = cube_lod_select<false>(rc, rho2, nb->lvl);
    }
    return cube_lod_finish(rc, fid, qs, qt, lod, nb->lvl);
}
__device__ __forceinline__ float cube_sample_lod_quad(const RenderConsts &rc, float px, float py, float pz, const QuadNb *nb) {
    const float qx = rc.cov_rot[0] * px + rc.cov_rot[2] * pz, qz = rc.cov_rot[1] * px + rc.cov_rot[3] * pz;
    const V3 d = {qx, py, qz};
    const float fid = __builtin_amdgcn_cubeid(qx, py, qz);
    const float sc = __builtin_amdgcn_cubesc(qx, py, qz);
    const float tc = __builtin_amdgcn_cubetc(qx, py, qz);
    const float ma2x = __builtin_amdgcn_cubema(qx, py, qz);
    const float ma = 0.5f * fabsf(ma2x);
    float qs, qt;
    cube_exact_quotients(sc, tc, ma, qs, qt);
    if (cube_lod_level0_certain(rc, qs, qt, ma, nb->e2)) return cube_lod_level0(rc, fid, qs, qt, nb->lvl);
    QuadRegs &q = *nb->regs;
    quad_exchange_coords(px, py, pz, rc.cov_rot[0], rc.cov_rot[1], rc.cov_rot[2], rc.cov_rot[3], q);
    if (!rc.cube_lod_fast)
        return cube_sample_lod(rc, d, nb->vx, cube_dir_from_coords(q.fidx, q.scx, q.tcx, q.masx), nb->vy, cube_dir_from_coords(q.fidy, q.scy, q.tcy, q.masy), nb->lvl);
    const float nf = (float)rc.cube_n, n2q = 0.25f * (nf * nf);
    constexpr bool EXACT = ATMO_LOD_LAMBDA_EXACT != 0;
    float rho2 = cube_lod_partner_coords<EXACT>(fid, sc, tc, ma2x, ma, d, nb->vx, q.fidx, q.scx, q.tcx, q.masx, n2q, 0.0f);
    rho2 = cube_lod_partner_coords<EXACT>(fid, sc, tc, ma2x, ma, d, nb->vy, q.fidy, q.scy, q.tcy, q.masy, n2q, rho2);
    return cube_lod_finish(rc, fid, qs, qt, cube_lod_select<EXACT>(rc, rho2, nb->lvl), nb->lvl);
}

struct LightMarchConsts {
    float ninv_h, c1, dens2, ratm2, inv_light_steps;
    int light_steps;
    float dens2_8;
};
#ifndef ATMO_LIGHT_FOLD
#define ATMO_LIGHT_FOLD 2
#endif
template <int LSTEPS>
__device__ __forceinline__ float sun_od_direct(const LightMarchConsts &k, float r2, float bdot, float y3) {
#pragma clang fp contract(fast)
    const float ninv_h = k.ninv_h, c1 = k.c1, dens2 = k.dens2, ratm2 = k.ratm2, inv_light_steps = k.inv_light_steps;
    const int light_steps = k.light_steps;
    const float hh = ratm2 - (r2 - bdot * bdot);
    const float sq = hw_sqrt((ATMO_LIGHT_FOLD >= 2 && LSTEPS == 8) ? hh : fmaxf(hh, 0.0f));
    const float ray_len = fmaxf(fminf(sq + sq, sq - bdot), 0.0f);
    const float lstep = ray_len * inv_light_steps;
    float acc = y3;
    if (LSTEPS == 8) {
        constexpr bool FOLD = ATMO_LIGHT_FOLD != 0;
        const float lb = FOLD ? ray_len * bdot : lstep * (bdot + bdot), l2 = FOLD ? ray_len * ray_len : lstep * lstep;
        constexpr float kb = FOLD ? 0.25f : 1.0f, k2 = FOLD ? 0.015625f : 1.0f;
        float q[8], rr[8];
#pragma unroll
        for (int j = 1; j < 8; ++j) q[j] = fmaf((float)(j * j) * k2, l2, fmaf((float)j * kb, lb, r2));
        asm volatile("v_sqrt_f32 %0, %7\n\tv_sqrt_f32 %1, %8\n\tv_sqrt_f32 %2, %9\n\tv_sqrt_f32 %3, %10\n\t"
                     "v_sqrt_f32 %4, %11\n\tv_sqrt_f32 %5, %12\n\tv_sqrt_f32 %6, %13\n\ts_nop 0"
                     : "=&v"(rr[1]), "=&v"(rr[2]), "=&v"(rr[3]), "=&v"(rr[4]), "=&v"(rr[5]), "=&v"(rr[6]), "=&v"(rr[7])
                     : "v"(q[1]), "v"(q[2]), "v"(q[3]), "v"(q[4]), "v"(q[5]), "v"(q[6]), "v"(q[7]));
#pragma unroll
        for (int j = 1; j < 8; ++j) {
            const float yy = sat(fmaf(rr[j], ninv_h, c1));
            acc = fmaf(yy * yy, yy, acc);
        }
        if (FOLD) return acc * ray_len * k.dens2_8;
    } else if (LSTEPS > 0) {
        const float lb = lstep * (bdot + bdot), l2 = lstep * lstep;
#pragma unroll
        for (int j = 1; j < (LSTEPS > 0 ? LSTEPS : 1); ++j) {
            const float rr = hw_sqrt(fmaf((float)(j * j), l2, fmaf((float)j, lb, r2)));
            const float yy = sat(fmaf(rr, ninv_h, c1));
            acc = fmaf(yy * yy, yy, acc);
        }
    } else {
        const float b2 = bdot + bdot;
        float sl = lstep;
        for (int j = 1; j < light_steps; ++j) {
            const float rr = hw_sqrt(fmaf(sl, sl + b2, r2));
            const float yy = sat(fmaf(rr, ninv_h, c1));
            acc = fmaf(yy * yy, yy, acc);
            sl += lstep;
        }
    }
    return acc * lstep * dens2;
}

__device__ __forceinline__ V3 scale_unfused(V3 d, float s) { return V3{d.x * s, d.y * s, d.z * s}; }
template <bool DIRECT, int LSTEPS, int SPLIT, bool VIEWPOS = false>
__device__ __forceinline__ float4 march_atmosphere(const RenderConsts &rc, V3 dir, float t_begin, float step_len, float jitter, int half) {
#pragma clang fp contract(fast)
    const int n0 = SPLIT == 2 ? (rc.view_steps + 1) / 2 : rc.view_steps;
    const int first = (SPLIT == 2 && half) ? n0 : 0;
    const int steps = (SPLIT == 2 && half) ? rc.view_steps - n0 : n0;
    t_begin = SPLIT == 2 ? fmaf((float)first, step_len, t_begin) : t_begin;
    const float inv_h = hw_rcp(rc.atmosphere_height);
    const float ninv_h = -inv_h;
    const float c1 = fmaf(rc.planet_radius, inv_h, 1.0f);
    const float dens2 = rc.density * rc.density;
    const float kr = -rc.coeff[0] * LOG2E, kg = -rc.coeff[1] * LOG2E, kb = -rc.coeff[2] * LOG2E;
    const float sx = rc.sun_dir[0], sy = rc.sun_dir[1], sz = rc.sun_dir[2];
    const float ratm2 = rc.atmosphere_radius * rc.atmosphere_radius;
    const int light_steps = LSTEPS > 0 ? LSTEPS : rc.light_steps;
    const float inv_light_steps = LSTEPS > 0 ? 1.0f / (float)(LSTEPS > 0 ? LSTEPS : 1) : hw_rcp((float)light_steps);
    const LightMarchConsts lmc = {ninv_h, c1, dens2, ratm2, inv_light_steps, light_steps, dens2 * 0.125f};
    const float half_w = 0.5f * (float)rc.lut_w, x_off = half_w - 0.5f;
    const float lut_hf = (float)rc.lut_h, y_off = lut_hf - 0.5f;

    static_assert(!VIEWPOS || SPLIT == 1, "reference-form position accumulation: one lane per ray");
    const V3 p0 = scale_unfused(dir, t_begin), sd = scale_unfused(dir, step_len);
    float pvx = p0.x, pvy = p0.y, pvz = p0.z;
    float ox = fmaf(dir.x, t_begin, -rc.center[0]);
    float oy = fmaf(dir.y, t_begin, -rc.center[1]);
    float oz = fmaf(dir.z, t_begin, -rc.center[2]);
    const float sdx = VIEWPOS ? sd.x : dir.x * step_len, sdy = VIEWPOS ? sd.y : dir.y * step_len, sdz = VIEWPOS ? sd.z : dir.z * step_len;
    const float dstep = dens2 * step_len;
    float lr = 0.0f, lg = 0.0f, lb = 0.0f, view_od = 0.0f;

#ifndef ATMO_LOOP_PAD
#define ATMO_LOOP_PAD 0
#endif
#if ATMO_LOOP_PAD > 0
#define ATMO_STR2(x) #x
#define ATMO_STR(x) ATMO_STR2(x)
    if (DIRECT && LSTEPS == 8 && SPLIT == 1 && !VIEWPOS) asm volatile(".rept " ATMO_STR(ATMO_LOOP_PAD) "\n\ts_nop 0\n\t.endr");
#endif
    for (int i = 0; i < steps; ++i) {
        if (VIEWPOS) {
            ox = pvx - rc.center[0]; oy = pvy - rc.center[1]; oz = pvz - rc.center[2];
        }
        const float r2 = ox * ox + oy * oy + oz * oz;
        const float bdot = ox * sx + oy * sy + oz * sz;
        const float inv_r = DIRECT ? 0.0f : hw_rsq(r2);
        const float r = DIRECT ? hw_sqrt(r2) : r2 * inv_r;
        const float y = sat(fmaf(r, ninv_h, c1));
        const float y3 = y * y * y;

        float sun_od;
        if (DIRECT) {
            sun_od = sun_od_direct<LSTEPS>(lmc, r2, bdot, y3);
        } else {
            const float x = fmaf(bdot * inv_r, half_w, x_off);
            const float yv = fmaf(-y, lut_hf, y_off);
            sun_od = lut_sample_fp(rc.lut4, rc.lut_w + 1, rc.lut_h + 1, x, yv);
        }

        const float d = y3 * dstep;
        view_od += d;
        const float od = sun_od + view_od;
        {
            const float ar = od * kr, ag = od * kg, ab = od * kb;
            float er, eg, eb;
            asm volatile("v_exp_f32 %0, %3\n\tv_exp_f32 %1, %4\n\tv_exp_f32 %2, %5\n\ts_nop 0" : "=&v"(er), "=&v"(eg), "=&v"(eb) : "v"(ar), "v"(ag), "v"(ab));
            lr = fmaf(d, er, lr);
            lg = fmaf(d, eg, lg);
            lb = fmaf(d, eb, lb);
        }

        if (VIEWPOS) {
            pvx += sdx; pvy += sdy; pvz += sdz;
        } else {
            ox += sdx; oy += sdy; oz += sdz;
        }
    }

    if (SPLIT == 2) {
        const float od_b = swap_adjacent(view_od), lr_b = swap_adjacent(lr), lg_b = swap_adjacent(lg), lb_b = swap_adjacent(lb);
        lr = fmaf(lr_b, hw_exp2(view_od * kr), lr);
        lg = fmaf(lg_b, hw_exp2(view_od * kg), lg);
        lb = fmaf(lb_b, hw_exp2(view_od * kb), lb);
        view_od += od_b;
    }
    const float alpha = 1.0f - hw_exp2(-view_od * LOG2E);
    float4 o;
    o.x = sat(fmaf(lr, rc.coeff[0], rc.ambient[0])) * rc.modulate[0];
    o.y = sat(fmaf(lg, rc.coeff[1], rc.ambient[1])) * rc.modulate[1];
    o.z = sat(fmaf(lb, rc.coeff[2], rc.ambient[2])) * rc.modulate[2];
    o.w = clampf(fmaf(jitter, 0.02f, alpha), 0.0f, 0.99f);
    return o;
}

template <int SPLIT>
__device__ __forceinline__ float4 march_atmosphere_v1(const RenderConsts &rc, V3 dir, float t_begin, float t_end, int half) {
#pragma clang fp contract(fast)
    const float inv_steps = 1.0f / (float)rc.view_steps;
    const float step_len = (t_end - t_begin) * inv_steps;
    const int n0 = SPLIT == 2 ? (rc.view_steps + 1) / 2 : rc.view_steps;
    const int steps = (SPLIT == 2 && half) ? rc.view_steps - n0 : n0;
    t_begin = (SPLIT == 2 && half) ? fmaf((float)n0, step_len, t_begin) : t_begin;
    const float inv_h = hw_rcp(rc.atmosphere_height);
    const float ninv_h = -inv_h;
    const float c1 = fmaf(rc.planet_radius, inv_h, 1.0f);
    const float sx = rc.sun_dir[0], sy = rc.sun_dir[1], sz = rc.sun_dir[2];
    float ox = fmaf(dir.x, t_begin, -rc.center[0]);
    float oy = fmaf(dir.y, t_begin, -rc.center[1]);
    float oz = fmaf(dir.z, t_begin, -rc.center[2]);
    const float sdx = dir.x * step_len, sdy = dir.y * step_len, sdz = dir.z * step_len;
    const float nds = -rc.density * step_len;
    float factor = 1.0f, light_sum = 0.0f;
    for (int i = 0; i < steps; ++i) {
        const float r2 = ox * ox + oy * oy + oz * oz;
        const float inv_r = hw_rsq(r2);
        const float y = sat(fmaf(r2 * inv_r, ninv_h, c1));
        const float cosang = (ox * sx + oy * sy + oz * sz) * inv_r;
        const float l = sat(fmaf(1.2f, cosang, 0.5f));
        light_sum = fmaf(l, l, light_sum);
        factor *= fmaf(y * y * y, nds, 1.0f);
        ox += sdx; oy += sdy; oz += sdz;
// ... 610 lines not shown
                           ieee_div((float)(w >> 30), 3.0f));
    } else {
        return *(const float4 *)p;
    }
}
template <int FMT>
__device__ __forceinline__ void target_encode(void *p, const float4 &v) {
    if constexpr (FMT == TF_RGBA16F) {
        *(uint2 *)p = make_uint2(half_bits_rne(v.x) | (half_bits_rne(v.y) << 16), half_bits_rne(v.z) | (half_bits_rne(v.w) << 16));
    } else if constexpr (FMT == TF_RGBA8_UNORM) {
        *(uint32_t *)p = unorm8_rne(v.x) | (unorm8_rne(v.y) << 8) | (unorm8_rne(v.z) << 16) | (unorm8_rne(v.w) << 24);
    } else if constexpr (tf_bytes4<FMT>) {
        const float c0 = tf_bgra<FMT> ? v.z : v.x, c2 = tf_bgra<FMT> ? v.x : v.z;
        if constexpr (tf_srgb<FMT>) *(uint32_t *)p = srgb8_encode(c0) | (srgb8_encode(v.y) << 8) | (srgb8_encode(c2) << 16) | (unorm8_rne(v.w) << 24);
        else *(uint32_t *)p = unorm8_rne(c0) | (unorm8_rne(v.y) << 8) | (unorm8_rne(c2) << 16) | (unorm8_rne(v.w) << 24);
    } else if constexpr (FMT == TF_A2B10G10R10_UNORM) {
        *(uint32_t *)p = unorm_rne<1023>(v.x) | (unorm_rne<1023>(v.y) << 10) | (unorm_rne<1023>(v.z) << 20) | (unorm_rne<3>(v.w) << 30);
    } else {
        *(float4 *)p = v;
    }
}
template <int FMT>
__device__ __forceinline__ void store_target(void *p, const float4 &src, const bool composite) {
    float4 o = src;
    if (composite) {
#pragma clang fp contract(off)
        const float4 dst = target_decode<FMT>(p);
        const float ia = 1.0f - src.w;
        o.x = src.x * src.w + dst.x * ia;
        o.y = src.y * src.w + dst.y * ia;
        o.z = src.z * src.w + dst.z * ia;
        o.w = src.w + dst.w * ia;
    }
    target_encode<FMT>(p, o);
}
__device__ __forceinline__ void store_target_rt(const int format, void *p, const float4 &src, const bool composite) {
    if (format == TF_RGBA16F) store_target<TF_RGBA16F>(p, src, composite);
    else if (format == TF_RGBA8_UNORM) store_target<TF_RGBA8_UNORM>(p, src, composite);
    else {
        int newer = format;
        asm volatile("" : "+s"(newer));
        if (newer == TF_RGBA8_SRGB) store_target<TF_RGBA8_SRGB>(p, src, composite);
        else if (newer == TF_BGRA8_SRGB) store_target<TF_BGRA8_SRGB>(p, src, composite);
        else if (newer == TF_BGRA8_UNORM) store_target<TF_BGRA8_UNORM>(p, src, composite);
        else store_target<TF_A2B10G10R10_UNORM>(p, src, composite);
    }
}
__device__ __forceinline__ void store_target_zero_rt(const int format, void *p) {
    if (format == TF_RGBA16F) *(uint2 *)p = make_uint2(0u, 0u);
    else *(uint32_t *)p = 0u;
}
__device__ __forceinline__ int target_pixel_shift_all(const int format) { return format == TF_RGBA32F ? 4 : (format == TF_RGBA16F ? 3 : 2); }
__device__ __forceinline__ void store_target_all_rt(const int format, void *p, const float4 &src, const bool composite) {
    if (format == TF_RGBA32F) store_target<TF_RGBA32F>(p, src, composite);
    else store_target_rt(format, p, src, composite);
}
__device__ __forceinline__ void store_target_zero_all_rt(const int format, void *p) {
    if (format == TF_RGBA32F) *(float4 *)p = make_float4(0.0f, 0.0f, 0.0f, 0.0f);
    else store_target_zero_rt(format, p);
}

template <int FLAGS, int LSTEPS, int SPLIT>
__device__ __forceinline__ void shade_pixel(const RenderConsts &rc, const int tile_x, const int tile_y, const ProxyConsts *pc = nullptr,
                                            const TargetConsts *tc = nullptr, const DepthConsts *dc = nullptr) {
    constexpr bool CLOUDS = (FLAGS & KF_CLOUDS) != 0;
    constexpr bool RM = (FLAGS & KF_CLOUD_LIGHT_RM) != 0;
    constexpr bool DIRECT = (FLAGS & KF_LIGHT_DIRECT) != 0;
    constexpr bool LITE = (FLAGS & KF_LITE) != 0;
    constexpr bool PRECISE = (FLAGS & KF_PRECISE) != 0;
    constexpr bool LOD = (FLAGS & KF_CUBE_LOD) != 0;
    constexpr bool ATMO_REF = (FLAGS & KF_ATMO_REF) != 0;
    constexpr bool VIEWPOS = (FLAGS & KF_VIEW_POS) != 0;
    constexpr bool PROXY = (FLAGS & KF_PROXY) != 0;
    constexpr bool TARGET = (FLAGS & KF_TARGET) != 0;
    constexpr bool DEPTH = (FLAGS & KF_DEPTH) != 0;
    static_assert(!DEPTH || TARGET, "depth sources: the target kernels' forms");
    static_assert(!TARGET || (!VIEWPOS && !ATMO_REF && (SPLIT == 1 || (FLAGS & KF_CUBE_LOD) != 0)),
                  "packed targets: the default forms; two lanes per ray only as the heavy-tile form of the declared-sampler cloud kernels");
    static_assert(!VIEWPOS || (!LITE && !ATMO_REF && SPLIT == 1), "KF_VIEW_POS: the fast v2 march, one lane per ray");
    static_assert(!PROXY || (!VIEWPOS && !ATMO_REF && SPLIT == 1 && (FLAGS & KF_GEO) == 0), "proxy draws: the default forms, one lane per ray, row-major");
    static_assert((FLAGS & KF_VIEWS) == 0 || (!VIEWPOS && !ATMO_REF && SPLIT == 1 && (FLAGS & KF_GEO) == 0),
                  "multi-view draws: the default forms, one lane per ray, float or packed targets (KF_VIEWS | KF_TARGET: atmo_render_views_target_kernel)");
    constexpr bool DIET = (!DIRECT || (ATMO_DIRECT_PROLOGUE_DIET && !CLOUDS)) && !((FLAGS & KF_CLOUDS) && (FLAGS & KF_CLOUD_LIGHT_RM));
    constexpr bool FASTMISS = (ATMO_FAST_MISS_MASK >> ((DIRECT ? 1 : 0) + (CLOUDS ? 2 : 0) + (LITE ? 4 : 0))) & 1;
    static_assert(!LOD || (CLOUDS && PRECISE), "implicit cubemap LOD: precise cloud kernels");
    static_assert(!(LOD && SPLIT == 2) || (!ATMO_REF && !VIEWPOS && !LITE && !DIRECT), "two lanes per ray under the declared sampler: the two BASELINE cloud kernels");
    static_assert(!LOD || (WAVE_W == 16 && WAVE_H == 4), "the quad-major lane order of the LOD kernels is written for 16 x 4 pixel waves");

    const int wave = threadIdx.x / 64, lane = threadIdx.x % 64;
    const f32x4 *lvl_table = nullptr;
    if constexpr (LOD) {
        __shared__ f32x4 lvl_lds[CUBE_LEVEL_TABLE + LOG2CR_ROWS];
        cube_level_table_fill(rc, lvl_lds, lane);
        log2_cr_table_fill(lvl_lds + CUBE_LEVEL_TABLE, lane);
        lvl_table = lvl_lds;
    }
    const int ray = SPLIT == 2 ? (LOD ? ((lane >> 3) << 2) | (lane & 3) : lane >> 1) : lane;
    const int half = SPLIT == 2 ? (LOD ? (lane >> 2) & 1 : lane & 1) : 0;
    constexpr int ASPLIT = LOD ? 1 : SPLIT;
    const int ahalf = LOD ? 0 : half;
    constexpr int WAVES_X = TILE_W / (WAVE_W > TILE_W ? TILE_W : WAVE_W);
    constexpr int WAVE_ROWS = WAVE_H / SPLIT;
    const int lx = (wave % WAVES_X) * WAVE_W + (LOD ? ((ray >> 2) & 7) * 2 + (ray & 1) : ray % WAVE_W);
    const int ly = (wave / WAVES_X) * WAVE_ROWS + (LOD ? ((ray >> 5) & 1) * 2 + ((ray >> 1) & 1) : ray / WAVE_W);
    const int px = (LOD ? rc.gx0 : rc.x0) + tile_x * TILE_W + lx;
    const int py = (LOD ? rc.gy0 : rc.y0) + tile_y * (TILE_H / SPLIT) + ly;
    QuadRegs qregs;
    if constexpr (LOD) quad_regs_define(qregs);
    if (LOD ? (px >= rc.w || py >= rc.h) : (px >= rc.x1 || py >= rc.y1)) return;
    bool helper = LOD && (px < rc.x0 || py < rc.y0 || px >= rc.x1 || py >= rc.y1);
    if constexpr (PROXY) {
        const bool pass = proxy_fragment_passes<DEPTH>(*pc, rc, px, py, dc);
        if constexpr (LOD) {
            const unsigned long long drawn = __builtin_amdgcn_ballot_w64(pass && !helper);
            if (((drawn >> (lane & ~3)) & 0xFull) == 0) return;
            helper = helper || !pass;
        } else {
            if (!pass) return;
        }
    }
    float4 *out = nullptr;
    char *tout = nullptr;
    if constexpr (DEPTH)
        tout = (char *)tc->pixels + (size_t)(py - rc.out_y0) * (size_t)tc->pitch_bytes + ((size_t)(px - rc.out_x0) << target_pixel_shift_all(tc->format));
    else if constexpr (TARGET)
        tout = (char *)tc->pixels + (size_t)(py - rc.out_y0) * (size_t)tc->pitch_bytes + ((size_t)(px - rc.out_x0) << (tc->format == TF_RGBA16F ? 3 : 2));
    else
        out = rc.out + (size_t)(py - rc.out_y0) * (size_t)rc.out_pitch + (px - rc.out_x0);

    if (FASTMISS && rc.miss_k > 0.0f) {
#pragma clang fp contract(fast)
        const float fnx = fmaf((float)px + 0.5f, rc.rcp_vw + rc.rcp_vw, -1.0f), fny = fmaf((float)py + 0.5f, rc.rcp_vh + rc.rcp_vh, -1.0f);
        const float *Q = rc.inv_p;
        const float ax = fmaf(Q[0], fnx, fmaf(Q[4], fny, Q[12]));
        const float ay = fmaf(Q[1], fnx, fmaf(Q[5], fny, Q[13]));
        const float az = fmaf(Q[2], fnx, fmaf(Q[6], fny, Q[14]));
        const float cv = rc.center[0] * ax + rc.center[1] * ay + rc.center[2] * az;
        const float vv = ax * ax + ay * ay + az * az;
        if (cv * cv < rc.miss_k * vv) {
            if (rc.store_discards && half == 0 && !helper) {
                if constexpr (DEPTH) store_target_zero_all_rt(tc->format, tout);
                else if constexpr (TARGET) store_target_zero_rt(tc->format, tout);
                else *out = make_float4(0.0f, 0.0f, 0.0f, 0.0f);
            }
            return;
        }
    }

    float nonlinear_depth;
    if constexpr (DEPTH) nonlinear_depth = load_depth(*dc, px, py);
    else nonlinear_depth = rc.depth[(size_t)py * rc.w + px];
    const float uvx = pixel_coord<DIET>((float)px + 0.5f, rc.vw, rc.rcp_vw);
    const float uvy = pixel_coord<DIET>((float)py + 0.5f, rc.vh, rc.rcp_vh);
    const float nx = uvx * 2.0f - 1.0f, ny = uvy * 2.0f - 1.0f, nz = nonlinear_depth;
    const float *P = rc.inv_p;
    const float vx = P[0] * nx + P[4] * ny + P[8] * nz + P[12] * 1.0f;
    const float vy = P[1] * nx + P[5] * ny + P[9] * nz + P[13] * 1.0f;
    const float vz = P[2] * nx + P[6] * ny + P[10] * nz + P[14] * 1.0f;
    const float vw = P[3] * nx + P[7] * ny + P[11] * nz + P[15] * 1.0f;
    const float *Vm = rc.inv_v;
    const float wx = Vm[0] * vx + Vm[4] * vy + Vm[8] * vz + Vm[12] * vw;
    const float wy = Vm[1] * vx + Vm[5] * vy + Vm[9] * vz + Vm[13] * vw;
    const float wz = Vm[2] * vx + Vm[6] * vy + Vm[10] * vz + Vm[14] * vw;
    const float ww = Vm[3] * vx + Vm[7] * vy + Vm[11] * vz + Vm[15] * vw;
    float pwx, pwy, pwz;
    world_div3<DIET>(wx, wy, wz, ww, pwx, pwy, pwz);
    const float ddx = rc.cam_pos_world[0] - pwx, ddy = rc.cam_pos_world[1] - pwy, ddz = rc.cam_pos_world[2] - pwz;
    float linear_depth = prologue_sqrt<DIET>(ddx * ddx + ddy * ddy + ddz * ddz);

    const float vvx = vx - 0.0f, vvy = vy - 0.0f, vvz = vz - 0.0f;
    const float inv_len = ieee_div(1.0f, prologue_sqrt<DIET>(vvx * vvx + vvy * vvy + vvz * vvz));
    const V3 dir = {vvx * inv_len, vvy * inv_len, vvz * inv_len};
    const V3 center = {rc.center[0], rc.center[1], rc.center[2]};

    const SphereHit sh = sphere_setup(center, dir);
    const float2 rs_atmo = hit_radius<DIET>(sh, rc.atmosphere_radius);

    if (rs_atmo.x == rs_atmo.y) {
        if (rc.store_discards && half == 0 && !helper) {
            if constexpr (DEPTH) store_target_zero_all_rt(tc->format, tout);
            else if constexpr (TARGET) store_target_zero_rt(tc->format, tout);
            else *out = make_float4(0.0f, 0.0f, 0.0f, 0.0f);
        }
        return;
    }
    const float t_begin = fmaxf(rs_atmo.x, 0.0f);
    float t_end = fmaxf(rs_atmo.y, 0.0f);
    const float2 rs_ground = hit_radius<DIET>(sh, rc.planet_radius);
    float gd = 10000000.0f;
    if (rs_ground.x != rs_ground.y) gd = rs_ground.x;
    linear_depth = linear_depth * (1.0f - rc.sphere_depth_factor) + gd * rc.sphere_depth_factor;
    t_end = fminf(t_end, linear_depth);

    const float jx = rc.vw * uvx, jy = rc.vh * uvy;
    const int ji = ((int)jx) & 0xff, jj = ((int)jy) & 0xff;
    const float jitter = blue_noise_value<DIET>(rc.blue[jj * 256 + ji]);

    float4 rgba;
    if (LITE) {
        if constexpr (PRECISE) rgba = march_atmosphere_v1_precise(rc, dir, t_begin, t_end);
        else rgba = march_atmosphere_v1<ASPLIT>(rc, dir, t_begin, t_end, ahalf);
    } else {
        if constexpr (ATMO_REF && SPLIT == 1) {
            rgba = march_atmosphere_v2_precise<DIRECT>(rc, dir, t_begin, t_end, jitter);
        } else {
            const float view_step_len = ieee_div(t_end - t_begin, (float)rc.view_steps);
            rgba = march_atmosphere<DIRECT, LSTEPS, ASPLIT, VIEWPOS>(rc, dir, t_begin, view_step_len, jitter, ahalf);
        }
    }

    if (CLOUDS) {
        const float2 rs_top = hit_radius<DIET>(sh, rc.clouds_top);
        if (rs_top.x != rs_top.y) {
            const float2 rs_bottom = hit_radius<DIET>(sh, rc.clouds_bottom);
            const float c0 = fmaxf(rs_top.x, 0.0f);
            const float c1 = fminf(rs_top.y, linear_depth);
            if (c0 < linear_depth && (linear_depth > rs_bottom.y || rs_bottom.x > 0.0f)) {
                const float *M = rc.view_to_model;
                V3 dir_m;
                dir_m.x = M[0] * dir.x + M[4] * dir.y + M[8] * dir.z;
                dir_m.y = M[1] * dir.x + M[5] * dir.y + M[9] * dir.z;
                dir_m.z = M[2] * dir.x + M[6] * dir.y + M[10] * dir.z;
                float2 rr;
                if constexpr (RM && SPLIT == 1 && !LOD) {
                    __shared__ float rmq[(TILE_W * TILE_H / 64) * RMQ_WORDS_PER_WAVE];
                    rr = march_clouds_rm_queue<PRECISE>(rc, dir_m, c0, c1, jitter, rmq + wave * RMQ_WORDS_PER_WAVE);
                } else {
                    rr = march_clouds<RM, PRECISE, SPLIT, LOD>(rc, dir_m, c0, c1, jitter, half, &qregs, lvl_table);
                }
                {
#pragma clang fp contract(fast)
                    const float cl = rr.x, ca = rr.y;
                    const float sa = 1.0f - ca;
                    const float a = rgba.w * sa + ca;
                    float abx = 0.0f, aby = 0.0f, abz = 0.0f, abw = 0.0f;
                    if (a != 0.0f) {
                        const float inv_a = ieee_div(1.0f, a);
                        const float ws = rgba.w * sa, wo = cl * ca;
                        abx = (rgba.x * ws + wo) * inv_a;
                        aby = (rgba.y * ws + wo) * inv_a;
                        abz = (rgba.z * ws + wo) * inv_a;
                        abw = a;
                    }
                    const float addx = rgba.x + cl * ca, addy = rgba.y + cl * ca, addz = rgba.z + cl * ca;
                    const float addw = fmaxf(rgba.w, ca);
                    rgba.x = mixf(abx, addx, rc.cloud_blend);
                    rgba.y = mixf(aby, addy, rc.cloud_blend);
                    rgba.z = mixf(abz, addz, rc.cloud_blend);
                    rgba.w = mixf(abw, addw, rc.cloud_blend);
                }
            }
        }
    }
    if constexpr (TARGET) {
        if (!(SPLIT == 2 && half) && !helper) {
            if constexpr (DEPTH) store_target_all_rt(tc->format, tout, rgba, rc.composite != 0);
            else store_target_rt(tc->format, tout, rgba, rc.composite != 0);
        }
        if constexpr (LOD) quad_regs_keep(qregs);
        return;
    }
    if constexpr (LOD) quad_regs_keep(qregs);
    if (SPLIT == 2 && half) return;
    if (helper) return;
    if (rc.composite) {
#pragma clang fp contract(off)
        const float4 dst = *out;
        const float ia = 1.0f - rgba.w;
        float4 o;
        o.x = rgba.x * rgba.w + dst.x * ia;
        o.y = rgba.y * rgba.w + dst.y * ia;
        o.z = rgba.z * rgba.w + dst.z * ia;
        o.w = rgba.w + dst.w * ia;
        *out = o;
    } else {
        *out = rgba;
    }
}

#ifndef ATMO_MIN_WAVES
#define ATMO_MIN_WAVES 6
#endif
#ifndef ATMO_MIN_WAVES_LOD_RM
#define ATMO_MIN_WAVES_LOD_RM 4
#endif
#ifndef ATMO_MIN_WAVES_LOD
#define ATMO_MIN_WAVES_LOD ATMO_MIN_WAVES
#endif
constexpr int render_min_waves(int flags) {
    return (flags & KF_CUBE_LOD) ? ((flags & KF_CLOUD_LIGHT_RM) ? ATMO_MIN_WAVES_LOD_RM : ATMO_MIN_WAVES_LOD) : ATMO_MIN_WAVES;
}
#if ATMO_MIN_WAVES > 0
#define ATMO_MIN_WAVES_ARG , render_min_waves(FLAGS)
#else
#define ATMO_MIN_WAVES_ARG
#endif
#ifndef ATMO_SGPR_CAP_VALUE
#define ATMO_SGPR_CAP_VALUE 80
#endif
#ifndef ATMO_SGPR_CAP_MASK
#define ATMO_SGPR_CAP_MASK 0x00
#endif
constexpr bool render_sgpr_cap80(int flags) {
    return (ATMO_SGPR_CAP_MASK >> (((flags & KF_LIGHT_DIRECT) ? 1 : 0) + ((flags & KF_CLOUDS) ? 2 : 0) + ((flags & KF_LITE) ? 4 : 0))) & 1;
}

#ifdef ATMO_WAVE_TRACE
#define ATMO_TRACE_ENTRY const uint64_t trace_entry = __builtin_amdgcn_s_memrealtime();
#define ATMO_SHADE_TRACED(TARGET, DEPTH)                                                                                           \
    const uint64_t trace_t0 = __builtin_amdgcn_s_memrealtime();                                                                    \
    shade_pixel<FLAGS, LSTEPS, SPLIT>(rc, (int)tile_x, (int)tile_y, nullptr, TARGET, DEPTH);                                       \
    if (rc.wave_trace != nullptr && (threadIdx.x & 63) == 0) {                                                                     \
        const uint32_t slot = (blockIdx.y * gridDim.x + blockIdx.x) * (TILE_W * TILE_H / 64) + (threadIdx.x >> 6);                 \
        unsigned long long *w = rc.wave_trace + 4ull * slot;                                                                       \
        w[0] = trace_t0;                                                                                                           \
        w[1] = __builtin_amdgcn_s_memrealtime();                                                                                   \
        w[2] = __builtin_amdgcn_s_getreg((31 << 11) | 4);                                               \
        w[3] = (__builtin_amdgcn_s_getreg((31 << 11) | 20) & 0xFu) | ((trace_t0 - trace_entry) << 8);  \
    }
#else
#define ATMO_TRACE_ENTRY
#define ATMO_SHADE_TRACED(TARGET, DEPTH) shade_pixel<FLAGS, LSTEPS, SPLIT>(rc, (int)tile_x, (int)tile_y, nullptr, TARGET, DEPTH);
#endif
__device__ __forceinline__ uint32_t geo_tile(const RenderConsts &rc, uint32_t b) {
    const uint32_t rows = (uint32_t)rc.geo_rows, tx = (uint32_t)rc.tiles_x, total = rc.geo_prefix[rows];
    if (b < total) {
        uint32_t lo = rc.geo_hint[0][b >> 8], hi = min((uint32_t)rc.geo_hint[0][(b >> 8) + 1] + 1u, rows);
        while (hi - lo > 1) {
            const uint32_t mid = (lo + hi) >> 1;
            if (rc.geo_prefix[mid] <= b) lo = mid; else hi = mid;
        }
        return lo * tx + rc.geo_first[lo] + (b - rc.geo_prefix[lo]);
    }
    const uint32_t m = b - total;
    uint32_t lo = rc.geo_hint[1][m >> 8], hi = min((uint32_t)rc.geo_hint[1][(m >> 8) + 1] + 1u, rows);
    while (hi - lo > 1) {
        const uint32_t mid = (lo + hi) >> 1;
        if (mid * tx - rc.geo_prefix[mid] <= m) lo = mid; else hi = mid;
    }
    const uint32_t o = m - (lo * tx - rc.geo_prefix[lo]), first = rc.geo_first[lo], len = rc.geo_prefix[lo + 1] - rc.geo_prefix[lo];
    return lo * tx + (o < first ? o : o + len);
}
#ifndef ATMO_LOOP_PAD_GEO
#define ATMO_LOOP_PAD_GEO 5
#endif
#define ATMO_PAD_STR2(x) #x
#define ATMO_PAD_STR(x) ATMO_PAD_STR2(x)
#define ATMO_HEAD_PAD(N) asm volatile(".rept " ATMO_PAD_STR(N) "\n\ts_nop 0\n\t.endr")
#define ATMO_RENDER_KERNEL_BODY(TARGET, DEPTH)                                                                   \
    ATMO_TRACE_ENTRY                                                                                             \
    uint32_t tile = blockIdx.y * gridDim.x + blockIdx.x;                                                         \
    if constexpr ((FLAGS & KF_GEO) != 0) {    \
        tile = geo_tile(rc, tile);                                                                               \
         \
        ATMO_HEAD_PAD(ATMO_LOOP_PAD_GEO);                                                                        \
    }                                                                                                            \
    if (rc.tile_order != nullptr) tile = rc.tile_order[tile];                                                    \
    const uint32_t tile_y = tile / (uint32_t)rc.tiles_x, tile_x = tile - tile_y * (uint32_t)rc.tiles_x;          \
    uint64_t t0 = 0;                                                                                             \
    if (rc.tile_cost != nullptr) t0 = __builtin_amdgcn_s_memtime();                                              \
    ATMO_SHADE_TRACED(TARGET, DEPTH)                                                                             \
    if (rc.tile_cost != nullptr && (threadIdx.x & 63) == 0) {                                                    \
        uint64_t dt = __builtin_amdgcn_s_memtime() - t0;                                                         \
        uint32_t cost_tile = tile;                                                                               \
        if constexpr (SPLIT == 2 && (FLAGS & KF_CUBE_LOD) != 0) {                                                \
             \
             \
            if (rc.cost_rows_halved) {                                                                           \
                cost_tile = (tile_y >> 1) * (uint32_t)rc.tiles_x + tile_x;                                       \
                dt *= 2;                                                                                         \
            }                                                                                                    \
        }                                                                                                        \
        atomicMax(&rc.tile_cost[cost_tile], (uint32_t)(dt > 0xffffffffull ? 0xffffffffull : dt));                \
    }

template <int FLAGS, int LSTEPS, int SPLIT = 1>
__global__ __launch_bounds__(TILE_W *TILE_H ATMO_MIN_WAVES_ARG) void atmo_render_kernel(const RenderConsts rc) {
    ATMO_RENDER_KERNEL_BODY(nullptr, nullptr)
}
template <int FLAGS, int LSTEPS>
__global__ __launch_bounds__(TILE_W *TILE_H ATMO_MIN_WAVES_ARG) void atmo_render_proxy_kernel(const RenderConsts rc, const ProxyConsts pc) {
    static_assert((FLAGS & KF_PROXY) != 0, "proxy kernels carry KF_PROXY");
    shade_pixel<FLAGS, LSTEPS, 1>(rc, (int)blockIdx.x, (int)blockIdx.y, &pc);
}
#ifndef ATMO_LOOP_PAD_VIEWS
#define ATMO_LOOP_PAD_VIEWS 3
#endif
constexpr int views_min_waves(int flags) {
    return ((flags & KF_CLOUDS) && !(flags & (KF_CLOUD_LIGHT_RM | KF_CUBE_LOD))) ? 8 : render_min_waves(flags);
}
#define ATMO_VIEWS_ORDERED_0(...)
#define ATMO_VIEWS_ORDERED_1(...) __VA_ARGS__
#define ATMO_VIEWS_KERNEL_BODY(V, ORDERED, PROXY, TARGET, DEPTH)                                                                       \
    uint32_t tile = blockIdx.x;                                                                                                        \
    ATMO_VIEWS_ORDERED_##ORDERED(if (V.order != nullptr) tile = V.order[tile];)                                                        \
    uint32_t view = 0;  \
    _Pragma("unroll") for (int i = 1; i < MAX_VIEWS; ++i) view += tile >= V.first_block[i] ? 1u : 0u;                                  \
    view = __builtin_amdgcn_readfirstlane(view);                                                                                       \
    const RenderConsts &rc = table[view];                                                                                              \
    const uint32_t local = tile - V.first_block[view];                                                                                 \
    const uint32_t tile_y = local / (uint32_t)rc.tiles_x, tile_x = local - tile_y * (uint32_t)rc.tiles_x;                              \
    ATMO_VIEWS_ORDERED_##ORDERED(uint64_t t0 = 0; if (V.cost != nullptr) t0 = __builtin_amdgcn_s_memtime();)                           \
    shade_pixel<FLAGS, LSTEPS, 1>(rc, (int)tile_x, (int)tile_y, PROXY, TARGET, DEPTH);                                                 \
    ATMO_VIEWS_ORDERED_##ORDERED(if (V.cost != nullptr && (threadIdx.x & 63) == 0) {                                                   \
        const uint64_t dt = __builtin_amdgcn_s_memtime() - t0;                                                                         \
        atomicMax(&V.cost[tile], (uint32_t)(dt > 0xffffffffull ? 0xffffffffull : dt));                                                 \
    })
template <int FLAGS, int LSTEPS>
__global__ __launch_bounds__(TILE_W *TILE_H, views_min_waves(FLAGS)) void atmo_render_views_kernel(const RenderConsts *__restrict__ table, const ViewsConsts vc) {
    static_assert((FLAGS & KF_VIEWS) != 0, "multi-view kernels carry KF_VIEWS");
    if constexpr (FLAGS == (KF_VIEWS | KF_LIGHT_DIRECT) && LSTEPS == 8) ATMO_HEAD_PAD(ATMO_LOOP_PAD_VIEWS);
    ATMO_VIEWS_KERNEL_BODY(vc, 1, nullptr, nullptr, nullptr)
}
template <int FLAGS, int LSTEPS, int SPLIT = 1>
__global__ __launch_bounds__(TILE_W *TILE_H ATMO_MIN_WAVES_ARG) __attribute__((amdgpu_num_sgpr(ATMO_SGPR_CAP_VALUE))) void atmo_render_kernel_s80(const RenderConsts rc) {
    ATMO_RENDER_KERNEL_BODY(nullptr, nullptr)
}

#ifndef ATMO_LOOP_PAD_TARGET
#define ATMO_LOOP_PAD_TARGET 3
#endif
#ifndef ATMO_LOOP_PAD_TARGET_GEO
#define ATMO_LOOP_PAD_TARGET_GEO 6
#endif
template <int FLAGS, int LSTEPS, int SPLIT = 1>
__global__ __launch_bounds__(TILE_W *TILE_H ATMO_MIN_WAVES_ARG) void atmo_render_target_kernel(const RenderConsts rc, const TargetConsts tc) {
    static_assert((FLAGS & KF_TARGET) != 0, "target kernels carry KF_TARGET");
    if constexpr ((FLAGS & ~KF_GEO) == (KF_TARGET | KF_LIGHT_DIRECT) && LSTEPS == 8 && SPLIT == 1) ATMO_HEAD_PAD(ATMO_LOOP_PAD_TARGET);
    if constexpr (FLAGS == (KF_TARGET | KF_LIGHT_DIRECT | KF_GEO) && LSTEPS == 8 && SPLIT == 1) ATMO_HEAD_PAD(ATMO_LOOP_PAD_TARGET_GEO);
    ATMO_RENDER_KERNEL_BODY(&tc, nullptr)
}
template <int FLAGS, int LSTEPS>
__global__ __launch_bounds__(TILE_W *TILE_H ATMO_MIN_WAVES_ARG) void atmo_render_proxy_target_kernel(const RenderConsts rc, const ProxyConsts pc,
                                                                                                      const TargetConsts tc) {
    static_assert((FLAGS & KF_PROXY) != 0 && (FLAGS & KF_TARGET) != 0, "proxy target kernels carry KF_PROXY | KF_TARGET");
    shade_pixel<FLAGS, LSTEPS, 1>(rc, (int)blockIdx.x, (int)blockIdx.y, &pc, &tc);
}
#ifndef ATMO_LOOP_PAD_VIEWS_TARGET
#define ATMO_LOOP_PAD_VIEWS_TARGET 3
#endif
template <int FLAGS, int LSTEPS>
__global__ __launch_bounds__(TILE_W *TILE_H, views_min_waves(FLAGS)) void atmo_render_views_target_kernel(const RenderConsts *__restrict__ table,
                                                                                                         const ViewsTargetConsts vtc) {
    static_assert((FLAGS & KF_VIEWS) != 0 && (FLAGS & KF_TARGET) != 0, "multi-view target kernels carry KF_VIEWS | KF_TARGET");
    if constexpr (FLAGS == (KF_VIEWS | KF_TARGET | KF_LIGHT_DIRECT) && LSTEPS == 8) ATMO_HEAD_PAD(ATMO_LOOP_PAD_VIEWS_TARGET);
    ATMO_VIEWS_KERNEL_BODY(vtc.v, 1, nullptr, &vtc.target[view], nullptr)
}
template <int FLAGS, int LSTEPS>
__global__ __launch_bounds__(TILE_W *TILE_H, views_min_waves(FLAGS)) void atmo_render_views_proxy_kernel(const RenderConsts *__restrict__ table,
                                                                                                        const ViewsProxyConsts vpc) {
    static_assert((FLAGS & KF_VIEWS) != 0 && (FLAGS & KF_PROXY) != 0 && (FLAGS & KF_TARGET) == 0, "multi-view proxy kernels carry KF_VIEWS | KF_PROXY");
    ATMO_VIEWS_KERNEL_BODY(vpc, 0, &vpc.proxy[view], nullptr, nullptr)
}
template <int FLAGS, int LSTEPS>
__global__ __launch_bounds__(TILE_W *TILE_H, views_min_waves(FLAGS)) void atmo_render_views_proxy_target_kernel(const RenderConsts *__restrict__ table,
                                                                                                               const ViewsProxyTargetConsts vptc) {
    static_assert((FLAGS & KF_VIEWS) != 0 && (FLAGS & KF_PROXY) != 0 && (FLAGS & KF_TARGET) != 0,
                  "multi-view proxy target kernels carry KF_VIEWS | KF_PROXY | KF_TARGET");
    ATMO_VIEWS_KERNEL_BODY(vptc.p, 0, &vptc.p.proxy[view], &vptc.target[view], nullptr)
}

constexpr int ORDER_BLOCKS = 256, ORDER_CLASSES = TILE_ORDER_CLASSES;
constexpr int ORDER_SUB_BITS = TILE_ORDER_PER_OCTAVE == 4 ? 2 : 1, ORDER_KEY_BITS = 4 + ORDER_SUB_BITS;
__device__ __forceinline__ uint32_t tile_cost_class(uint32_t c) {
    if (c == 0) return ORDER_CLASSES - 1;
    const int msb = 31 - __builtin_clz(c);
    const int q = msb * TILE_ORDER_PER_OCTAVE + (msb >= ORDER_SUB_BITS ? (int)((c >> (msb - ORDER_SUB_BITS)) & (uint32_t)(TILE_ORDER_PER_OCTAVE - 1)) : 0) - 8 * TILE_ORDER_PER_OCTAVE;
    return (uint32_t)(ORDER_CLASSES - 1 - (q < 0 ? 0 : (q > ORDER_CLASSES - 1 ? ORDER_CLASSES - 1 : q)));
}
__device__ __forceinline__ unsigned long long match_class(uint32_t key, bool valid) {
    unsigned long long m = __builtin_amdgcn_ballot_w64(valid);
#pragma unroll
    for (int bit = 0; bit < ORDER_KEY_BITS; ++bit) {
        const bool one = (key >> bit) & 1u;
        const unsigned long long b = __builtin_amdgcn_ballot_w64(one);
        m &= one ? b : ~b;
    }
    return m;
}
__device__ __forceinline__ int lanes_below(unsigned long long m) {
    return (int)__builtin_amdgcn_mbcnt_hi((uint32_t)(m >> 32), __builtin_amdgcn_mbcnt_lo((uint32_t)m, 0u));
}

__global__ __launch_bounds__(64) void atmo_tile_hist_kernel(const uint32_t *__restrict__ cost, uint32_t *__restrict__ hist, int n) {
    __shared__ uint32_t cnt[ORDER_CLASSES];
    const int lane = threadIdx.x, chunk = (n + ORDER_BLOCKS - 1) / ORDER_BLOCKS;
    const int i0 = min((int)blockIdx.x * chunk, n), i1 = min(i0 + chunk, n);
    if (lane < ORDER_CLASSES) cnt[lane] = 0;
    __syncthreads();
    for (int i = i0; i < i1; i += 64) {
        const bool valid = i + lane < i1;
        const uint32_t c = valid ? tile_cost_class(cost[i + lane]) : 0u;
        const unsigned long long m = match_class(c, valid);
        if (valid && lanes_below(m) == 0) cnt[c] += (uint32_t)__builtin_popcountll(m);
    }
    __syncthreads();
    if (lane < ORDER_CLASSES) hist[lane * ORDER_BLOCKS + blockIdx.x] = cnt[lane];
}

__global__ __launch_bounds__(256) void atmo_tile_scan_kernel(uint32_t *__restrict__ hist, uint32_t *__restrict__ class_totals) {
    __shared__ uint32_t total[ORDER_CLASSES];
    const int lane = threadIdx.x & 63, wave = threadIdx.x >> 6;
    constexpr int PER_LANE = ORDER_BLOCKS / 64, PER_WAVE = ORDER_CLASSES / 4;
    uint32_t excl_keep[PER_WAVE][PER_LANE];
#pragma unroll
    for (int q = 0; q < PER_WAVE; ++q) {
        const int c = wave * PER_WAVE + q;
        uint32_t sum = 0;
#pragma unroll
        for (int k = 0; k < PER_LANE; ++k) {
            excl_keep[q][k] = sum;
            sum += hist[c * ORDER_BLOCKS + lane * PER_LANE + k];
        }
        uint32_t incl = sum;
#pragma unroll
        for (int d = 1; d < 64; d <<= 1) {
            const uint32_t x = __shfl_up(incl, d);
            if (lane >= d) incl += x;
        }
#pragma unroll
        for (int k = 0; k < PER_LANE; ++k) excl_keep[q][k] += incl - sum;
        if (lane == 63) total[c] = incl;
// ... 593 lines not shown
    return launch_default_family(flags, light_steps, [&](auto F, auto L) -> hipError_t {
        return launch_batch(atmo_render_views_proxy_target_kernel<F | KF_VIEWS | KF_PROXY | KF_TARGET, L>, vptc.p.first_block, table, stream, vptc);
    });
}

template <int FMT>
__global__ __launch_bounds__(256) void atmo_store_target_kernel(const float4 *__restrict__ src, void *dst, size_t n, int composite) {
    const size_t i = (size_t)blockIdx.x * blockDim.x + threadIdx.x;
    if (i >= n) return;
    constexpr size_t BYTES = FMT == TF_RGBA32F ? 16 : (FMT == TF_RGBA16F ? 8 : 4);
    store_target<FMT>((char *)dst + i * BYTES, src[i], composite != 0);
}
hipError_t launch_store_target(int format, int composite, const float *src_rgba, void *dst, size_t n, hipStream_t stream) {
    if (n == 0) return hipSuccess;
    if (n > ((size_t)1 << 31)) return hipErrorInvalidValue;
    const dim3 grid((unsigned)((n + 255) / 256)), block(256);
    const float4 *src = (const float4 *)src_rgba;
    switch (format) {
    case TF_RGBA32F: hipLaunchKernelGGL(atmo_store_target_kernel<TF_RGBA32F>, grid, block, 0, stream, src, dst, n, composite); break;
    case TF_RGBA16F: hipLaunchKernelGGL(atmo_store_target_kernel<TF_RGBA16F>, grid, block, 0, stream, src, dst, n, composite); break;
    case TF_RGBA8_UNORM: hipLaunchKernelGGL(atmo_store_target_kernel<TF_RGBA8_UNORM>, grid, block, 0, stream, src, dst, n, composite); break;
    case TF_RGBA8_SRGB: hipLaunchKernelGGL(atmo_store_target_kernel<TF_RGBA8_SRGB>, grid, block, 0, stream, src, dst, n, composite); break;
    case TF_BGRA8_UNORM: hipLaunchKernelGGL(atmo_store_target_kernel<TF_BGRA8_UNORM>, grid, block, 0, stream, src, dst, n, composite); break;
    case TF_BGRA8_SRGB: hipLaunchKernelGGL(atmo_store_target_kernel<TF_BGRA8_SRGB>, grid, block, 0, stream, src, dst, n, composite); break;
    case TF_A2B10G10R10_UNORM: hipLaunchKernelGGL(atmo_store_target_kernel<TF_A2B10G10R10_UNORM>, grid, block, 0, stream, src, dst, n, composite); break;
    default: return hipErrorInvalidValue;
    }
    return hipGetLastError();
}

const char *render_kernel_name(int flags, int light_steps, int split) {
    static thread_local char name[80];
    const bool v2_precise = (flags & KF_ATMO_REF) != 0;
    const int lsteps = ((flags & KF_LIGHT_DIRECT) && light_steps == 8 && !v2_precise && !(flags & KF_VIEW_POS)) ? 8 : 0;
    if (flags & KF_DEPTH) {
        const char *views = (flags & KF_VIEWS) ? "_views" : "", *proxy = (flags & KF_PROXY) ? "_proxy" : "";
        if (flags & (KF_VIEWS | KF_PROXY)) snprintf(name, sizeof(name), "atmo_render%s%s_depth_target_kernel<%d, %d>", views, proxy, flags, lsteps);
        else snprintf(name, sizeof(name), "atmo_render_depth_target_kernel<%d, %d, %d>", flags, lsteps, split == 2 ? 2 : 1);
        return name;
    }
    if ((flags & KF_VIEWS) && (flags & KF_PROXY)) {
        snprintf(name, sizeof(name), "atmo_render_views_proxy%s_kernel<%d, %d>", (flags & KF_TARGET) ? "_target" : "", flags, lsteps);
        return name;
    }
    if (flags & KF_PROXY) {
        snprintf(name, sizeof(name), "atmo_render_proxy%s_kernel<%d, %d>", (flags & KF_TARGET) ? "_target" : "", flags, lsteps);
        return name;
    }
    if (flags & KF_VIEWS) {
        snprintf(name, sizeof(name), "atmo_render_views%s_kernel<%d, %d>", (flags & KF_TARGET) ? "_target" : "", flags, lsteps);
        return name;
    }
    if (flags & KF_TARGET) {
        snprintf(name, sizeof(name), "atmo_render_target_kernel<%d, %d, %d>", flags, lsteps, split == 2 ? 2 : 1);
        return name;
    }
    snprintf(name, sizeof(name), "atmo_render_kernel%s<%d, %d, %d>", render_sgpr_cap80(flags) ? "_s80" : "", flags, lsteps, split == 2 ? 2 : 1);
    return name;
}

__global__ void atmo_lut_footprint_kernel(const float *__restrict__ apron, int w, int h, float *__restrict__ out4) {
    const int i = blockIdx.x * blockDim.x + threadIdx.x, j = blockIdx.y;
    if (i > w || j > h) return;
    const int st = w + 2;
    const float *p = apron + (size_t)j * st + i;
    float *o = out4 + ((size_t)j * (w + 1) + i) * 4;
    o[0] = p[0]; o[1] = p[1]; o[2] = p[st]; o[3] = p[st + 1];
}
hipError_t launch_lut_footprints(const float *apron, int w, int h, float *out4, hipStream_t stream) {
    hipLaunchKernelGGL(atmo_lut_footprint_kernel, dim3((w + 1 + 255) / 256, h + 1), dim3(256), 0, stream, apron, w, h, out4);
    return hipGetLastError();
}

hipError_t launch_bake(const BakeConsts &bc, hipStream_t stream) {
    dim3 grid((bc.w + 15) / 16, (bc.h + 15) / 16);
    hipLaunchKernelGGL(atmo_bake_kernel, grid, dim3(256), 0, stream, bc);
    return hipGetLastError();
}

#ifndef ATMO_LOOP_PAD_DEPTH
#define ATMO_LOOP_PAD_DEPTH 2
#endif
#ifndef ATMO_LOOP_PAD_DEPTH_GEO
#define ATMO_LOOP_PAD_DEPTH_GEO 2
#endif
#ifndef ATMO_LOOP_PAD_DEPTH_VIEWS
#define ATMO_LOOP_PAD_DEPTH_VIEWS 0
#endif
template <int FLAGS, int LSTEPS, int SPLIT = 1>
__global__ __launch_bounds__(TILE_W *TILE_H ATMO_MIN_WAVES_ARG) void atmo_render_depth_target_kernel(const RenderConsts rc, const TargetConsts tc,
                                                                                                      const DepthConsts dc) {
    static_assert((FLAGS & KF_TARGET) != 0 && (FLAGS & KF_DEPTH) != 0, "depth-source kernels carry KF_DEPTH | KF_TARGET");
    if constexpr ((FLAGS & ~KF_GEO) == (KF_DEPTH | KF_TARGET | KF_LIGHT_DIRECT) && LSTEPS == 8 && SPLIT == 1) ATMO_HEAD_PAD(ATMO_LOOP_PAD_DEPTH);
    if constexpr (FLAGS == (KF_DEPTH | KF_TARGET | KF_LIGHT_DIRECT | KF_GEO) && LSTEPS == 8 && SPLIT == 1) ATMO_HEAD_PAD(ATMO_LOOP_PAD_DEPTH_GEO);
    ATMO_RENDER_KERNEL_BODY(&tc, &dc)
}
template <int FLAGS, int LSTEPS>
__global__ __launch_bounds__(TILE_W *TILE_H ATMO_MIN_WAVES_ARG) void atmo_render_proxy_depth_target_kernel(const RenderConsts rc, const ProxyConsts pc,
                                                                                                            const TargetConsts tc, const DepthConsts dc) {
    static_assert((FLAGS & KF_PROXY) != 0 && (FLAGS & KF_TARGET) != 0 && (FLAGS & KF_DEPTH) != 0, "KF_DEPTH | KF_PROXY | KF_TARGET");
    shade_pixel<FLAGS, LSTEPS, 1>(rc, (int)blockIdx.x, (int)blockIdx.y, &pc, &tc, &dc);
}
template <int FLAGS, int LSTEPS>
__global__ __launch_bounds__(TILE_W *TILE_H, views_min_waves(FLAGS)) void atmo_render_views_depth_target_kernel(const RenderConsts *__restrict__ table,
                                                                                                               const ViewsTargetConsts vtc,
                                                                                                               const ViewsDepthConsts vdc) {
    static_assert((FLAGS & KF_VIEWS) != 0 && (FLAGS & KF_TARGET) != 0 && (FLAGS & KF_DEPTH) != 0, "KF_DEPTH | KF_VIEWS | KF_TARGET");
    if constexpr (FLAGS == (KF_DEPTH | KF_VIEWS | KF_TARGET | KF_LIGHT_DIRECT) && LSTEPS == 8) ATMO_HEAD_PAD(ATMO_LOOP_PAD_DEPTH_VIEWS);
    ATMO_VIEWS_KERNEL_BODY(vtc.v, 1, nullptr, &vtc.target[view], &vdc.depth[view])
}
template <int FLAGS, int LSTEPS>
__global__ __launch_bounds__(TILE_W *TILE_H, views_min_waves(FLAGS)) void atmo_render_views_proxy_depth_target_kernel(
    const RenderConsts *__restrict__ table, const ViewsProxyTargetConsts vptc, const ViewsDepthConsts vdc) {
    static_assert((FLAGS & KF_VIEWS) != 0 && (FLAGS & KF_PROXY) != 0 && (FLAGS & KF_TARGET) != 0 && (FLAGS & KF_DEPTH) != 0,
                  "KF_DEPTH | KF_VIEWS | KF_PROXY | KF_TARGET");
    ATMO_VIEWS_KERNEL_BODY(vptc.p, 0, &vptc.p.proxy[view], &vptc.target[view], &vdc.depth[view])
}

hipError_t launch_render_depth_target(int flags, int split, const RenderConsts &rc, const TargetConsts &tc, const DepthConsts &dc, hipStream_t stream,
                                      int tile_list_blocks) {
    if (!target_format_known(tc.format) || !depth_consts_valid(dc) || !target_family_supported(flags & ~KF_GEO, split)) return hipErrorInvalidValue;
    return launch_default_family<true>(flags, rc.light_steps, [&](auto F, auto L) -> hipError_t {
        if constexpr (target_family_has_split(F)) {
            if (split == 2) return launch_tiles(atmo_render_depth_target_kernel<F | KF_DEPTH | KF_TARGET, L, 2>, 2, rc, tile_list_blocks, stream, tc, dc);
        }
        return launch_tiles(atmo_render_depth_target_kernel<F | KF_DEPTH | KF_TARGET, L, 1>, 1, rc, tile_list_blocks, stream, tc, dc);
    });
}
hipError_t launch_render_proxy_depth_target(int flags, const RenderConsts &rc, const ProxyConsts &pc, const TargetConsts &tc, const DepthConsts &dc,
                                            hipStream_t stream) {
    if (!target_format_known(tc.format) || !depth_consts_valid(dc)) return hipErrorInvalidValue;
    return launch_default_family(flags, rc.light_steps, [&](auto F, auto L) -> hipError_t {
        return launch_rect(atmo_render_proxy_depth_target_kernel<F | KF_DEPTH | KF_PROXY | KF_TARGET, L>, rc, stream, pc, tc, dc);
    });
}
hipError_t launch_render_views_depth_target(int flags, int light_steps, const RenderConsts *table, const ViewsTargetConsts &vtc, const ViewsDepthConsts &vdc,
                                            hipStream_t stream) {
    if (!batch_targets_valid(vtc.v.first_block, vtc.target, vdc.depth)) return hipErrorInvalidValue;
    return launch_default_family(flags, light_steps, [&](auto F, auto L) -> hipError_t {
        return launch_batch(atmo_render_views_depth_target_kernel<F | KF_DEPTH | KF_VIEWS | KF_TARGET, L>, vtc.v.first_block, table, stream, vtc, vdc);
    });
}
hipError_t launch_render_views_proxy_depth_target(int flags, int light_steps, const RenderConsts *table, const ViewsProxyTargetConsts &vptc,
                                                  const ViewsDepthConsts &vdc, hipStream_t stream) {
    if (!batch_targets_valid(vptc.p.first_block, vptc.target, vdc.depth)) return hipErrorInvalidValue;
    return launch_default_family(flags, light_steps, [&](auto F, auto L) -> hipError_t {
        return launch_batch(atmo_render_views_proxy_depth_target_kernel<F | KF_DEPTH | KF_VIEWS | KF_PROXY | KF_TARGET, L>, vptc.p.first_block, table,
                            stream, vptc, vdc);
    });
}

__global__ __launch_bounds__(256) void atmo_decode_depth_kernel(int format, const void *texels, float *__restrict__ out, size_t n) {
    const size_t i = (size_t)blockIdx.x * blockDim.x + threadIdx.x;
    if (i >= n) return;
    out[i] = depth_decode(format, (const char *)texels + (i << (format == DF_D16_UNORM ? 1 : 2)));
}
hipError_t launch_decode_depth(int format, const void *texels, float *out, size_t n, hipStream_t stream) {
    if (n == 0) return hipSuccess;
    if (n > ((size_t)1 << 31) || depth_texel_bytes(format) == 0) return hipErrorInvalidValue;
    hipLaunchKernelGGL(atmo_decode_depth_kernel, dim3((unsigned)((n + 255) / 256)), dim3(256), 0, stream, format, texels, out, n);
    return hipGetLastError();
}

}
```

Measured before the change: 25210 Mrays/s.

## Specialize ray prologue for standard camera matrices and host-precomputed constants

The host now detects frames whose inverse projection and view matrices have the usual sparse camera structure. For those frames the kernel uses a reduced matrix-vector form to build the ray, skips the ground-sphere intersection when sphere_depth_factor is zero, and multiplies by a precomputed reciprocal when the step count is a power of two. Squared radii, density squared and the log2e-scaled coefficients are also computed once on the host and passed in the constants, and the loop-padding nop counts are retuned across several kernels. The aim is to cut per-pixel prologue ALU work, at the cost of a wave-wide ballot check, extra branches and more constant-buffer fields.

```diff
diff --git a/godot_atmosphere_shader_amd/_native.py b/godot_atmosphere_shader_amd/_native.py
--- a/godot_atmosphere_shader_amd/_native.py
+++ b/godot_atmosphere_shader_amd/_native.py
@@ -37,6 +37,8 @@
 DEPTH_SYMBOLS = ("atmo_depth_texel_bytes", "atmo_render_depth_target", "atmo_render_proxy_depth_target", "atmo_render_views_depth_target",
                  "atmo_render_views_proxy_depth_target")
 DEPTH_D32_SFLOAT, DEPTH_D16_UNORM, DEPTH_X8_D24_UNORM = range(3)
+PROLOGUE_SYMBOLS = ("atmo_debug_prologue_mode", "atmo_debug_prologue_constants")
+PROLOGUE_CAMERA, PROLOGUE_POW2_STEPS, PROLOGUE_NO_SPHERE_DEPTH = 1, 2, 4
 EXPORTED_SYMBOLS = CORE_SYMBOLS + DEBUG_SYMBOLS + SCENE_SYMBOLS + TARGET_SYMBOLS + VIEWS_SYMBOLS + VIEWS_PROXY_SYMBOLS + VIEWS_TARGET_SYMBOLS
 TARGET_RGBA32F, TARGET_RGBA16F, TARGET_RGBA8_UNORM = range(3)
 TARGET_RGBA8_SRGB, TARGET_BGRA8_UNORM, TARGET_BGRA8_SRGB, TARGET_A2B10G10R10_UNORM = range(16, 20)
@@ -214,6 +216,8 @@
         "atmo_debug_tile_order": (ip, [vp, vp, ip, ip, ip, ip, vp, vp, vp, vp, C.POINTER(ip)]),
         "atmo_debug_heavy_tile_count": (ip, [vp, ip, ip, C.c_float, C.c_float, ip]),
         "atmo_debug_feedback_plan": (ip, [C.POINTER(AtmoFeedbackPlanIn), C.POINTER(AtmoFeedbackPlanOut)]),
+        "atmo_debug_prologue_mode": (ip, [vp, C.POINTER(AtmoFrame), C.POINTER(C.c_uint), C.POINTER(ip), C.POINTER(ip)]),
+        "atmo_debug_prologue_constants": (ip, [vp, C.POINTER(AtmoFrame), fp, ip, C.POINTER(ip)]),
     }
     ab_build = bool(os.environ.get("ATMO_HIP_LIB"))
     for name, (res, args) in sig.items():
diff --git a/godot_atmosphere_shader_amd/build.py b/godot_atmosphere_shader_amd/build.py
--- a/godot_atmosphere_shader_amd/build.py
+++ b/godot_atmosphere_shader_amd/build.py
@@ -12,7 +12,7 @@
            os.path.join("..", "..", "include", "atmo_scene.h"), os.path.join("..", "..", "include", "atmo_target.h"),
            os.path.join("..", "..", "include", "atmo_views.h"), os.path.join("..", "..", "include", "atmo_views_target.h"),
            os.path.join("..", "..", "include", "atmo_views_proxy.h"), os.path.join("..", "..", "include", "atmo_planets.h"),
-           os.path.join("..", "..", "include", "atmo_depth.h")]
+           os.path.join("..", "..", "include", "atmo_depth.h"), os.path.join("..", "..", "include", "atmo_debug_prologue.h")]
 
 HIPCC_FLAGS = ["--offload-arch=gfx950", "-O3", "-std=c++17", "-ffp-contract=off", "-fno-slp-vectorize", "-fPIC",
                "-shared", "-Wall", "-Wno-unused-function"]
diff --git a/godot_atmosphere_shader_amd/csrc/atmo_api.hip b/godot_atmosphere_shader_amd/csrc/atmo_api.hip
--- a/godot_atmosphere_shader_amd/csrc/atmo_api.hip
+++ b/godot_atmosphere_shader_amd/csrc/atmo_api.hip
@@ -7,6 +7,7 @@
 #include "../../include/atmo_views_proxy.h"
 #include "../../include/atmo_planets.h"
 #include "../../include/atmo_depth.h"
+#include "../../include/atmo_debug_prologue.h"
 #include "atmo_device.h"
 #include "atmo_layout.h"
 #include "atmo_feedback_plan.h"
@@ -174,6 +175,7 @@
     unsigned moving_period = 2;
     int f4_footprints = 3;
     int env_lod0_cert = 1;
+    int prologue_camera = 1;
     int instream = 1;
     int fb_axis_windows = 1;
     uint32_t *measure_cost = nullptr;
@@ -282,6 +284,41 @@
     return t * t * (3.0f - 2.0f * t);
 }
 
+static inline uint32_t f32_bits(float x) { uint32_t u; std::memcpy(&u, &x, sizeof(u)); return u; }
+static void prologue_camera_fill(const AtmoContext *ctx, atmo::RenderConsts &rc) {
+    constexpr float LOG2E = 1.44269504088896340736f;
+    rc.view_steps_f = (float)rc.view_steps;
+    rc.atmosphere_radius2 = rc.atmosphere_radius * rc.atmosphere_radius;
+    rc.planet_radius2 = rc.planet_radius * rc.planet_radius;
+    rc.dens2 = rc.density * rc.density;
+    rc.dens2_8 = rc.dens2 * 0.125f;
+    for (int i = 0; i < 3; ++i) rc.coeff_log2e[i] = -rc.coeff[i] * LOG2E;
+    rc.inv_view_steps = 0.0f;
+    rc.prologue_mode = 0;
+    rc.cam_skip_px = rc.cam_skip_py = -1;
+    if (!ctx->prologue_camera) return;
+    auto zero = [](float x) { return (f32_bits(x) & 0x7fffffffu) == 0u; };
+    auto minus_zero = [](float x) { return f32_bits(x) == 0x80000000u; };
+    auto bounded = [](float x) { return std::fabs(x) <= 0x1p40f; };
+    const float *P = rc.inv_p, *V = rc.inv_v;
+    bool cam = true;
+    for (int i : {1, 2, 3, 4, 6, 7, 8, 9, 10}) cam = cam && zero(P[i]);
+    cam = cam && zero(V[3]) && zero(V[7]) && zero(V[11]) && f32_bits(V[15]) == 0x3f800000u;
+    cam = cam && P[11] != 0.0f && std::fabs(P[0]) >= 0x1p-40f && std::fabs(P[5]) >= 0x1p-40f && std::fabs(P[14]) >= 0x1p-40f;
+    for (int i = 0; i < 16; ++i) cam = cam && bounded(P[i]) && bounded(V[i]);
+    for (int i = 0; i < 3; ++i) cam = cam && bounded(rc.center[i]);
+    cam = cam && bounded(rc.atmosphere_radius) && bounded(rc.planet_radius);
+    if (cam) rc.prologue_mode |= atmo::PM_CAMERA;
+    if (cam && minus_zero(P[12]) && P[0] < 0.0f && (rc.w & 1)) rc.cam_skip_px = rc.w / 2;
+    if (cam && minus_zero(P[13]) && P[5] < 0.0f && (rc.h & 1)) rc.cam_skip_py = rc.h / 2;
+    const int n = rc.view_steps;
+    if (n >= 1 && n <= (1 << 20) && (n & (n - 1)) == 0) {
+        rc.prologue_mode |= atmo::PM_POW2_STEPS;
+        rc.inv_view_steps = 1.0f / rc.view_steps_f;
+    }
+    if (cam && zero(rc.sphere_depth_factor)) rc.prologue_mode |= atmo::PM_NO_SPHERE_DEPTH;
+}
+
 void fill_consts(const AtmoContext *ctx, const AtmoFrame *f, const float *depth, float *rgba, atmo::RenderConsts &rc) {
     const Params &p = ctx->p;
     std::memset(&rc, 0, sizeof(rc));
@@ -423,6 +460,7 @@
     rc.store_discards = ctx->target_cleared ? 0 : 1;
     rc.gx0 = f->x0;
     rc.gy0 = f->y0;
+    prologue_camera_fill(ctx, rc);
 }
 
 int resolve_sampler_lod(const AtmoContext *ctx, const char **why_not) {
@@ -941,6 +979,7 @@
     if (const char *ev = std::getenv("ATMO_DRAW_EVENTS")) ctx->draw_events = ev[0] == '0' ? 0 : (ev[0] == '2' ? 2 : 1);
     if (const char *ev = std::getenv("ATMO_TARGET_CLEARED")) ctx->target_cleared = ev[0] == '1' ? 1 : 0;
     if (const char *ev = std::getenv("ATMO_GEO_ORDER")) ctx->geo_order = ev[0] == '0' ? 0 : 1;
+    if (const char *ev = std::getenv("ATMO_PROLOGUE_CAMERA")) ctx->prologue_camera = ev[0] == '0' ? 0 : 1;
     if (const char *ev = std::getenv("ATMO_FB_INSTREAM")) ctx->instream = ev[0] >= '1' && ev[0] <= '2' ? ev[0] - '0' : 0;
     if (const char *ev = std::getenv("ATMO_FB_AXIS_WINDOWS")) ctx->fb_axis_windows = ev[0] == '1' ? 1 : 0;
     if (const char *ev = std::getenv("ATMO_FB_REACH_SCALE")) ctx->env_reach_scale = (float)std::atof(ev);
@@ -1931,6 +1970,7 @@
     AtmoContext *ctx = new (std::nothrow) AtmoContext();
     if (!ctx) return fail(nullptr, ATMO_E_ARG, "atmo_debug_create_host_only: out of host memory");
     init_variant(ctx,  -1, variant, view_steps, cloud_steps, light_mode, light_steps);
+    if (const char *ev = std::getenv("ATMO_PROLOGUE_CAMERA")) ctx->prologue_camera = ev[0] == '0' ? 0 : 1;
     *out = ctx;
     return ATMO_OK;
 }
@@ -1962,6 +2002,34 @@
     return ATMO_OK;
 }
 
+int atmo_debug_prologue_mode(AtmoContext *ctx, const AtmoFrame *frame, unsigned int *mode, int *skip_px, int *skip_py) {
+    if (!ctx) return ATMO_E_ARG;
+    if (!frame || !mode) return fail(ctx, ATMO_E_ARG, "atmo_debug_prologue_mode: null argument");
+    AtmoFrame fixed;
+    atmo::RenderConsts rc;
+    fill_consts(ctx, draw_frame(ctx, frame, fixed), nullptr, nullptr, rc);
+    *mode = rc.prologue_mode;
+    if (skip_px) *skip_px = rc.cam_skip_px;
+    if (skip_py) *skip_py = rc.cam_skip_py;
+    return ATMO_OK;
+}
+
+int atmo_debug_prologue_constants(AtmoContext *ctx, const AtmoFrame *frame, float *out, int capacity, int *count) {
+    if (!ctx) return ATMO_E_ARG;
+    if (!frame) return fail(ctx, ATMO_E_ARG, "atmo_debug_prologue_constants: null frame");
+    AtmoFrame fixed;
+    atmo::RenderConsts rc;
+    fill_consts(ctx, draw_frame(ctx, frame, fixed), nullptr, nullptr, rc);
+    const float v[] = {rc.inv_view_steps, rc.view_steps_f, rc.atmosphere_radius2, rc.planet_radius2, rc.dens2, rc.dens2_8,
+                       rc.coeff_log2e[0], rc.coeff_log2e[1], rc.coeff_log2e[2],
+                       rc.atmosphere_radius, rc.planet_radius, rc.density, rc.coeff[0], rc.coeff[1], rc.coeff[2], rc.sphere_depth_factor};
+    const int n = (int)(sizeof(v) / sizeof(v[0]));
+    if (count) *count = n;
+    if (!out) return ATMO_OK;
+    if (capacity < n) return fail(ctx, ATMO_E_ARG, "atmo_debug_prologue_constants: buffer too small");
+    std::memcpy(out, v, sizeof(v));
+    return ATMO_OK;
+}
 
 static void mat4_mul_d(const double *a, const double *b, double *c) {
     for (int col = 0; col < 4; ++col)
diff --git a/godot_atmosphere_shader_amd/csrc/atmo_device.h b/godot_atmosphere_shader_amd/csrc/atmo_device.h
--- a/godot_atmosphere_shader_amd/csrc/atmo_device.h
+++ b/godot_atmosphere_shader_amd/csrc/atmo_device.h
@@ -80,6 +80,19 @@
     uint16_t geo_prefix[GEO_MAX_ROWS + 1];
     uint8_t geo_first[GEO_MAX_ROWS];
     uint16_t geo_hint[2][GEO_MAX_HINTS + 2];
+    uint32_t prologue_mode;
+    int32_t cam_skip_px, cam_skip_py;
+    float inv_view_steps;
+    float view_steps_f;
+    float atmosphere_radius2;
+    float planet_radius2;
+    float dens2, dens2_8;
+    float coeff_log2e[3];
+};
+enum PrologueMode : uint32_t {
+    PM_CAMERA = 1,
+    PM_POW2_STEPS = 2,
+    PM_NO_SPHERE_DEPTH = 4,
 };
 
 struct BakeConsts {
diff --git a/godot_atmosphere_shader_amd/csrc/atmo_kernels.hip b/godot_atmosphere_shader_amd/csrc/atmo_kernels.hip
--- a/godot_atmosphere_shader_amd/csrc/atmo_kernels.hip
+++ b/godot_atmosphere_shader_amd/csrc/atmo_kernels.hip
@@ -76,6 +76,14 @@
 #ifndef ATMO_DIRECT_PROLOGUE_DIET
 #define ATMO_DIRECT_PROLOGUE_DIET 1
 #endif
+#ifndef ATMO_PROLOGUE_CAMERA_FORMS
+#define ATMO_PROLOGUE_CAMERA_FORMS 15
+#endif
+__device__ __forceinline__ float uniform_in_vgpr(float s) {
+    float v;
+    asm("v_mov_b32 %0, %1" : "=v"(v) : "s"(s));
+    return v;
+}
 template <bool DIET = true>
 __device__ __forceinline__ float prologue_sqrt(float x) { return DIET ? exact_sqrt(x) : ieee_sqrt(x); }
 template <bool DIET = true>
@@ -136,6 +144,13 @@
 template <bool DIET = true>
 __device__ __forceinline__ float2 hit_radius(SphereHit s, float radius) {
     float h = radius * radius - s.qc2;
+    if (h < 0.0f) return make_float2(1000000.0f, 1000000.0f);
+    h = prologue_sqrt<DIET>(h);
+    return make_float2(-s.b - h, -s.b + h);
+}
+template <bool DIET = true>
+__device__ __forceinline__ float2 hit_radius2(SphereHit s, float radius2) {
+    float h = radius2 - s.qc2;
     if (h < 0.0f) return make_float2(1000000.0f, 1000000.0f);
     h = prologue_sqrt<DIET>(h);
     return make_float2(-s.b - h, -s.b + h);
@@ -846,7 +861,7 @@
 }
 
 __device__ __forceinline__ V3 scale_unfused(V3 d, float s) { return V3{d.x * s, d.y * s, d.z * s}; }
-template <bool DIRECT, int LSTEPS, int SPLIT, bool VIEWPOS = false>
+template <bool DIRECT, int LSTEPS, int SPLIT, bool VIEWPOS = false, bool HANDED = false>
 __device__ __forceinline__ float4 march_atmosphere(const RenderConsts &rc, V3 dir, float t_begin, float step_len, float jitter, int half) {
 #pragma clang fp contract(fast)
     const int n0 = SPLIT == 2 ? (rc.view_steps + 1) / 2 : rc.view_steps;
@@ -856,13 +871,15 @@
     const float inv_h = hw_rcp(rc.atmosphere_height);
     const float ninv_h = -inv_h;
     const float c1 = fmaf(rc.planet_radius, inv_h, 1.0f);
-    const float dens2 = rc.density * rc.density;
-    const float kr = -rc.coeff[0] * LOG2E, kg = -rc.coeff[1] * LOG2E, kb = -rc.coeff[2] * LOG2E;
+    const float dens2 = HANDED ? rc.dens2 : rc.density * rc.density;
+    const float kr = HANDED ? uniform_in_vgpr(rc.coeff_log2e[0]) : -rc.coeff[0] * LOG2E;
+    const float kg = HANDED ? uniform_in_vgpr(rc.coeff_log2e[1]) : -rc.coeff[1] * LOG2E;
+    const float kb = HANDED ? uniform_in_vgpr(rc.coeff_log2e[2]) : -rc.coeff[2] * LOG2E;
     const float sx = rc.sun_dir[0], sy = rc.sun_dir[1], sz = rc.sun_dir[2];
-    const float ratm2 = rc.atmosphere_radius * rc.atmosphere_radius;
+    const float ratm2 = HANDED ? uniform_in_vgpr(rc.atmosphere_radius2) : rc.atmosphere_radius * rc.atmosphere_radius;
     const int light_steps = LSTEPS > 0 ? LSTEPS : rc.light_steps;
     const float inv_light_steps = LSTEPS > 0 ? 1.0f / (float)(LSTEPS > 0 ? LSTEPS : 1) : hw_rcp((float)light_steps);
-    const LightMarchConsts lmc = {ninv_h, c1, dens2, ratm2, inv_light_steps, light_steps, dens2 * 0.125f};
+    const LightMarchConsts lmc = {ninv_h, c1, dens2, ratm2, inv_light_steps, light_steps, HANDED ? uniform_in_vgpr(rc.dens2_8) : dens2 * 0.125f};
     const float half_w = 0.5f * (float)rc.lut_w, x_off = half_w - 0.5f;
     const float lut_hf = (float)rc.lut_h, y_off = lut_hf - 0.5f;
 
@@ -877,12 +894,12 @@
     float lr = 0.0f, lg = 0.0f, lb = 0.0f, view_od = 0.0f;
 
 #ifndef ATMO_LOOP_PAD
-#define ATMO_LOOP_PAD 0
+#define ATMO_LOOP_PAD 5
 #endif
 #if ATMO_LOOP_PAD > 0
 #define ATMO_STR2(x) #x
 #define ATMO_STR(x) ATMO_STR2(x)
-    if (DIRECT && LSTEPS == 8 && SPLIT == 1 && !VIEWPOS) asm volatile(".rept " ATMO_STR(ATMO_LOOP_PAD) "\n\ts_nop 0\n\t.endr");
+    if (DIRECT && HANDED && LSTEPS == 8 && SPLIT == 1 && !VIEWPOS) asm volatile(".rept " ATMO_STR(ATMO_LOOP_PAD) "\n\ts_nop 0\n\t.endr");
 #endif
     for (int i = 0; i < steps; ++i) {
         if (VIEWPOS) {
@@ -1659,6 +1676,7 @@
     static_assert((FLAGS & KF_VIEWS) == 0 || (!VIEWPOS && !ATMO_REF && SPLIT == 1 && (FLAGS & KF_GEO) == 0),
                   "multi-view draws: the default forms, one lane per ray, float or packed targets (KF_VIEWS | KF_TARGET: atmo_render_views_target_kernel)");
     constexpr bool DIET = (!DIRECT || (ATMO_DIRECT_PROLOGUE_DIET && !CLOUDS)) && !((FLAGS & KF_CLOUDS) && (FLAGS & KF_CLOUD_LIGHT_RM));
+    constexpr int CAMF = (DIRECT && !CLOUDS && ATMO_DIRECT_PROLOGUE_DIET) ? ATMO_PROLOGUE_CAMERA_FORMS : 0;
     constexpr bool FASTMISS = (ATMO_FAST_MISS_MASK >> ((DIRECT ? 1 : 0) + (CLOUDS ? 2 : 0) + (LITE ? 4 : 0))) & 1;
     static_assert(!LOD || (CLOUDS && PRECISE), "implicit cubemap LOD: precise cloud kernels");
     static_assert(!(LOD && SPLIT == 2) || (!ATMO_REF && !VIEWPOS && !LITE && !DIRECT), "two lanes per ray under the declared sampler: the two BASELINE cloud kernels");
@@ -1731,15 +1749,34 @@
     const float uvy = pixel_coord<DIET>((float)py + 0.5f, rc.vh, rc.rcp_vh);
     const float nx = uvx * 2.0f - 1.0f, ny = uvy * 2.0f - 1.0f, nz = nonlinear_depth;
     const float *P = rc.inv_p;
-    const float vx = P[0] * nx + P[4] * ny + P[8] * nz + P[12] * 1.0f;
-    const float vy = P[1] * nx + P[5] * ny + P[9] * nz + P[13] * 1.0f;
-    const float vz = P[2] * nx + P[6] * ny + P[10] * nz + P[14] * 1.0f;
-    const float vw = P[3] * nx + P[7] * ny + P[11] * nz + P[15] * 1.0f;
     const float *Vm = rc.inv_v;
+    float vx, vy, vz, vw, ww;
+    bool cam = false;
+    if constexpr ((CAMF & 5) != 0) {
+        if (rc.prologue_mode & PM_CAMERA) {
+            const float vws = P[11] * nz + P[15];
+            cam = __builtin_amdgcn_ballot_w64(!__builtin_amdgcn_classf(vws, 0x198) || px == rc.cam_skip_px || py == rc.cam_skip_py) == 0ull;
+            if constexpr ((CAMF & 1) != 0) {
+                if (cam) {
+                    vx = P[0] * nx + P[12];
+                    vy = P[5] * ny + P[13];
+                    vz = P[14];
+                    vw = vws;
+                    ww = vws;
+                }
+            }
+        }
+    }
+    if ((CAMF & 1) == 0 || !cam) {
+        vx = P[0] * nx + P[4] * ny + P[8] * nz + P[12] * 1.0f;
+        vy = P[1] * nx + P[5] * ny + P[9] * nz + P[13] * 1.0f;
+        vz = P[2] * nx + P[6] * ny + P[10] * nz + P[14] * 1.0f;
+        vw = P[3] * nx + P[7] * ny + P[11] * nz + P[15] * 1.0f;
+        ww = Vm[3] * vx + Vm[7] * vy + Vm[11] * vz + Vm[15] * vw;
+    }
     const float wx = Vm[0] * vx + Vm[4] * vy + Vm[8] * vz + Vm[12] * vw;
     const float wy = Vm[1] * vx + Vm[5] * vy + Vm[9] * vz + Vm[13] * vw;
     const float wz = Vm[2] * vx + Vm[6] * vy + Vm[10] * vz + Vm[14] * vw;
-    const float ww = Vm[3] * vx + Vm[7] * vy + Vm[11] * vz + Vm[15] * vw;
     float pwx, pwy, pwz;
     world_div3<DIET>(wx, wy, wz, ww, pwx, pwy, pwz);
     const float ddx = rc.cam_pos_world[0] - pwx, ddy = rc.cam_pos_world[1] - pwy, ddz = rc.cam_pos_world[2] - pwz;
@@ -1751,7 +1788,9 @@
     const V3 center = {rc.center[0], rc.center[1], rc.center[2]};
 
     const SphereHit sh = sphere_setup(center, dir);
-    const float2 rs_atmo = hit_radius<DIET>(sh, rc.atmosphere_radius);
+    float2 rs_atmo;
+    if constexpr ((CAMF & 8) != 0) rs_atmo = hit_radius2<DIET>(sh, rc.atmosphere_radius2);
+    else rs_atmo = hit_radius<DIET>(sh, rc.atmosphere_radius);
 
     if (rs_atmo.x == rs_atmo.y) {
         if (rc.store_discards && half == 0 && !helper) {
@@ -1763,10 +1802,14 @@
     }
     const float t_begin = fmaxf(rs_atmo.x, 0.0f);
     float t_end = fmaxf(rs_atmo.y, 0.0f);
-    const float2 rs_ground = hit_radius<DIET>(sh, rc.planet_radius);
-    float gd = 10000000.0f;
-    if (rs_ground.x != rs_ground.y) gd = rs_ground.x;
-    linear_depth = linear_depth * (1.0f - rc.sphere_depth_factor) + gd * rc.sphere_depth_factor;
+    if (!((CAMF & 4) != 0 && cam && (rc.prologue_mode & PM_NO_SPHERE_DEPTH))) {
+        float2 rs_ground;
+        if constexpr ((CAMF & 8) != 0) rs_ground = hit_radius2<DIET>(sh, rc.planet_radius2);
+        else rs_ground = hit_radius<DIET>(sh, rc.planet_radius);
+        float gd = 10000000.0f;
+        if (rs_ground.x != rs_ground.y) gd = rs_ground.x;
+        linear_depth = linear_depth * (1.0f - rc.sphere_depth_factor) + gd * rc.sphere_depth_factor;
+    }
     t_end = fminf(t_end, linear_depth);
 
     const float jx = rc.vw * uvx, jy = rc.vh * uvy;
@@ -1781,8 +1824,10 @@
         if constexpr (ATMO_REF && SPLIT == 1) {
             rgba = march_atmosphere_v2_precise<DIRECT>(rc, dir, t_begin, t_end, jitter);
         } else {
-            const float view_step_len = ieee_div(t_end - t_begin, (float)rc.view_steps);
-            rgba = march_atmosphere<DIRECT, LSTEPS, ASPLIT, VIEWPOS>(rc, dir, t_begin, view_step_len, jitter, ahalf);
+            float view_step_len;
+            if ((CAMF & 2) != 0 && (rc.prologue_mode & PM_POW2_STEPS)) view_step_len = (t_end - t_begin) * rc.inv_view_steps;
+            else view_step_len = ieee_div(t_end - t_begin, (CAMF & 8) != 0 ? rc.view_steps_f : (float)rc.view_steps);
+            rgba = march_atmosphere<DIRECT, LSTEPS, ASPLIT, VIEWPOS, (CAMF & 8) != 0>(rc, dir, t_begin, view_step_len, jitter, ahalf);
         }
     }
 
@@ -1919,7 +1964,7 @@
     return lo * tx + (o < first ? o : o + len);
 }
 #ifndef ATMO_LOOP_PAD_GEO
-#define ATMO_LOOP_PAD_GEO 5
+#define ATMO_LOOP_PAD_GEO 7
 #endif
 #define ATMO_PAD_STR2(x) #x
 #define ATMO_PAD_STR(x) ATMO_PAD_STR2(x)
@@ -1961,7 +2006,7 @@
     shade_pixel<FLAGS, LSTEPS, 1>(rc, (int)blockIdx.x, (int)blockIdx.y, &pc);
 }
 #ifndef ATMO_LOOP_PAD_VIEWS
-#define ATMO_LOOP_PAD_VIEWS 3
+#define ATMO_LOOP_PAD_VIEWS 7
 #endif
 constexpr int views_min_waves(int flags) {
     return ((flags & KF_CLOUDS) && !(flags & (KF_CLOUD_LIGHT_RM | KF_CUBE_LOD))) ? 8 : render_min_waves(flags);
@@ -1998,7 +2043,7 @@
 #define ATMO_LOOP_PAD_TARGET 3
 #endif
 #ifndef ATMO_LOOP_PAD_TARGET_GEO
-#define ATMO_LOOP_PAD_TARGET_GEO 6
+#define ATMO_LOOP_PAD_TARGET_GEO 5
 #endif
 template <int FLAGS, int LSTEPS, int SPLIT = 1>
 __global__ __launch_bounds__(TILE_W *TILE_H ATMO_MIN_WAVES_ARG) void atmo_render_target_kernel(const RenderConsts rc, const TargetConsts tc) {
@@ -2014,7 +2059,7 @@
     shade_pixel<FLAGS, LSTEPS, 1>(rc, (int)blockIdx.x, (int)blockIdx.y, &pc, &tc);
 }
 #ifndef ATMO_LOOP_PAD_VIEWS_TARGET
-#define ATMO_LOOP_PAD_VIEWS_TARGET 3
+#define ATMO_LOOP_PAD_VIEWS_TARGET 7
 #endif
 template <int FLAGS, int LSTEPS>
 __global__ __launch_bounds__(TILE_W *TILE_H, views_min_waves(FLAGS)) void atmo_render_views_target_kernel(const RenderConsts *__restrict__ table,
@@ -2774,10 +2819,10 @@
 #define ATMO_LOOP_PAD_DEPTH 2
 #endif
 #ifndef ATMO_LOOP_PAD_DEPTH_GEO
-#define ATMO_LOOP_PAD_DEPTH_GEO 2
+#define ATMO_LOOP_PAD_DEPTH_GEO 3
 #endif
 #ifndef ATMO_LOOP_PAD_DEPTH_VIEWS
-#define ATMO_LOOP_PAD_DEPTH_VIEWS 0
+#define ATMO_LOOP_PAD_DEPTH_VIEWS 6
 #endif
 template <int FLAGS, int LSTEPS, int SPLIT = 1>
 __global__ __launch_bounds__(TILE_W *TILE_H ATMO_MIN_WAVES_ARG) void atmo_render_depth_target_kernel(const RenderConsts rc, const TargetConsts tc,
diff --git a/include/atmo_debug_prologue.h b/include/atmo_debug_prologue.h
--- /dev/null
+++ b/include/atmo_debug_prologue.h
@@ -0,0 +1,22 @@
+#ifndef ATMO_DEBUG_PROLOGUE_H
+#define ATMO_DEBUG_PROLOGUE_H
+
+#include "atmo.h"
+
+#ifdef __cplusplus
+extern "C" {
+#endif
+
+#define ATMO_PROLOGUE_CAMERA 1u
+#define ATMO_PROLOGUE_POW2_STEPS 2u
+#define ATMO_PROLOGUE_NO_SPHERE_DEPTH 4u
+
+int atmo_debug_prologue_mode(AtmoContext *ctx, const AtmoFrame *frame, unsigned int *mode, int *skip_px, int *skip_py);
+
+int atmo_debug_prologue_constants(AtmoContext *ctx, const AtmoFrame *frame, float *out, int capacity, int *count);
+
+#ifdef __cplusplus
+}
+#endif
+
+#endif
```

Measured after the change: 25640 Mrays/s, median of 6. 1.7% higher.
